# td-kwj-zp2023/webgpu-msm-bls12-377

Measured on AMD Instinct MI355X. Metric: ms per 2^20 BLS12-377 G1 MSM, lower is better.
Workload: dtype u32 (29-bit limbs, 64-bit accumulate)

## Files before the change

### webgpu-msm-bls12-377_amd/csrc/capi.hip

```cpp
#include <hip/hip_runtime.h>
#include <stdlib.h>
#include <string.h>

#include <algorithm>
#include <new>

#include "context.hpp"
#include "host_tail.hpp"
#include "sequencer.hpp"
#include "batch_mul_host.hpp"
#include "import_host.hpp"
#include "validate_host.hpp"

using namespace msm377;

#define HIP_TRY(ctx, call)                                                  \
  do {                                                                      \
    if (!eng::hip_ok((ctx), (int)(call), #call)) return MSM377_EHIP;        \
  } while (0)


extern "C" {

const char* msm377_version(void) { return "msm377 0.1 gfx950"; }

const char* msm377_strerror(int code) {
  switch (code) {
    case MSM377_OK: return "ok";
    case MSM377_EINVAL: return "invalid argument";
    case MSM377_EHIP: return "HIP runtime error";
    case MSM377_ESCALAR: return "scalar out of range for the signed window recode";
    case MSM377_ENOMEM: return "out of memory";
    case MSM377_ESTATE: return "call sequence error";
    case MSM377_EGLVRANGE: return "scalar outside the GLV range";
    case MSM377_EEXCEPTIONAL: return "exceptional case of the twisted Edwards law while combining partial records";
    case MSM377_EPOINT: return "an input point failed a requested check (canonical / on the curve / in the subgroup)";
    default: return "unknown error";
  }
}

int msm377_ctx_create(int device, uint64_t max_points, msm377_ctx** out) {
  if (!out || max_points == 0 || max_points > (1ull << 30)) return MSM377_EINVAL;
  *out = nullptr;
  int count = 0;
  if (hipGetDeviceCount(&count) != hipSuccess || device < 0 || device >= count) return MSM377_EHIP;
  msm377_ctx* ctx = new (std::nothrow) msm377_ctx();
  if (!ctx) return MSM377_ENOMEM;
  ctx->device = device;
  ctx->cap = max_points;
  if (const char* e = getenv("MSM377_GLV")) ctx->glv_mode = atoi(e);
  if (const char* e = getenv("MSM377_G1_FORM")) ctx->g1_form = atoi(e) != 0;
  if (const char* e = getenv("MSM377_CONV_WAVE_PRIO")) ctx->conv_wave_prio = atoi(e) != 0;
  if (const char* e = getenv("MSM377_AFF_PREWAKE_US")) ctx->aff_prewake_us = atoll(e);
  if (const char* e = getenv("MSM377_UPLOAD_CHUNKS")) ctx->upload_chunks = (uint32_t)std::min(std::max(atoi(e), 2), 7);
  if (const char* e = getenv("MSM377_UPLOAD_SPLIT")) ctx->upload_split_pct = (uint32_t)std::min(std::max(atoi(e), 5), 90);
  if (const char* e = getenv("MSM377_UPLOAD_CHUNK_MIN")) ctx->upload_chunk_min = strtoull(e, nullptr, 10);
  if (const char* e = getenv("MSM377_TAIL_THREADS")) ctx->tail_threads = std::min(std::max(atoi(e), 1), TailPool::WORKERS + 1);
  if (const char* e = getenv("MSM377_TAIL_WAIT_MS")) ctx->tail_pool.wait_limit_ns = (int64_t)std::max(atoi(e), 1) * 1000000ll;
  if (const char* e = getenv("MSM377_TAIL_SPIN_US")) ctx->tail_spin_us = atoll(e);
  if (const char* e = getenv("MSM377_TAIL_TRACE")) ctx->tail_trace = atoi(e) != 0;
  if (const char* e = getenv("MSM377_TAIL_NUMA")) ctx->tail_pool.numa_local = atoi(e) != 0;
  if (const char* e = getenv("MSM377_TE_AFFINE_MSM")) ctx->te_affine_msm = atoi(e) != 0;
  if (const char* e = getenv("MSM377_NARROW_MAX")) ctx->narrow_max_points = strtoull(e, nullptr, 10);
  if (const char* e = getenv("MSM377_PRECOMP_BITS")) ctx->precomp_bits = atoi(e) == (int)WIDE_BITS ? (int)WIDE_BITS : MSM377_WINDOW_BITS;
  if (const char* e = getenv("MSM377_AFFINE_MIN")) ctx->affine_min_points = strtoull(e, nullptr, 10);
  if (const char* e = getenv("MSM377_SEG_PLAIN")) ctx->seg_plain = std::min(std::max(atoi(e), (int)SEG_MIN), (int)SEG_MAX);
  if (const char* e = getenv("MSM377_SEG_GLV")) ctx->seg_glv = std::min(std::max(atoi(e), (int)SEG_MIN), (int)SEG_MAX);
  if (const char* e = getenv("MSM377_ZERO_COPY_OUT")) ctx->zc_out = atoi(e);
  if (const char* e = getenv("MSM377_NARROW_SEG")) ctx->narrow_seg = (uint32_t)std::min(std::max(atoi(e), (int)NARROW_SEG), (int)SEG_BINS - 1);
  if (const char* e = getenv("MSM377_NARROW_QUAD_ITEMS")) ctx->narrow_quad_items = strtoull(e, nullptr, 10);
  if (const char* e = getenv("MSM377_COOP_THREADS")) ctx->coop_threads = (uint32_t)atoi(e);
  if (const char* e = getenv("MSM377_NARROW_TAIL_FROM")) ctx->narrow_tail_from = (uint32_t)std::min(std::max(atoi(e), 1), (int)TREE_LEVELS);
  if (const char* e = getenv("MSM377_TAIL_LDS")) ctx->tail_lds = atoi(e) != 0;
  if (const char* e = getenv("MSM377_REDUCE_COLUMNS")) ctx->reduce_columns = atoi(e) != 0;
  if (const char* e = getenv("MSM377_EVEN_WINDOWS")) ctx->even_windows = atoi(e) != 0;
  if (const char* e = getenv("MSM377_SORT_ELEM")) ctx->sort_elem = atoi(e) == 4 ? 4u : 8u;
  if (const char* e = getenv("MSM377_TWIN_BATCH")) ctx->twin_batches = atoi(e) != 0;
  if (const char* e = getenv("MSM377_BASE_CHECKS")) ctx->base_checks = check_flags_normal((uint32_t)strtoul(e, nullptr, 0));
  if (const char* e = getenv("MSM377_TAIL_FROM")) ctx->tail_from = (uint32_t)std::min(std::max(atoi(e), 1), (int)TREE_LEVELS);
  const uint64_t cap = max_points;
  int prio_least = 0, prio_greatest = 0;
  bool ok = hipSetDevice(device) == hipSuccess;
  if (ok && hipDeviceGetStreamPriorityRange(&prio_least, &prio_greatest) != hipSuccess) prio_least = prio_greatest = 0;
  ok = ok && hipStreamCreateWithPriority(&ctx->stream, hipStreamNonBlocking, prio_greatest) == hipSuccess &&
            hipStreamCreateWithPriority(&ctx->stream2, hipStreamNonBlocking, prio_least) == hipSuccess &&
            hipEventCreateWithFlags(&ctx->bases_ready, hipEventDisableTiming) == hipSuccess;
  auto dalloc = [&](void** p, size_t bytes) { ok = ok && hipMalloc(p, bytes) == hipSuccess; };
  dalloc((void**)&ctx->d_raw_points, cap * 96);
  dalloc((void**)&ctx->d_raw_scalars, cap * 32);
  dalloc((void**)&ctx->d_bases, 2 * cap * G1_REC_WORDS * 4);
  const uint64_t wcap = std::max<uint64_t>((uint64_t)MSM377_NUM_WINDOWS * cap, (uint64_t)NARROW_EVEN_WINDOWS * std::min<uint64_t>(cap, SMALL_SORT_MAX));
  dalloc((void**)&ctx->d_digits, wcap * 2);
  dalloc((void**)&ctx->d_range_counts, (size_t)NRANGE * MAX_SORT_BLOCKS * 4);
  dalloc((void**)&ctx->d_region_base, (size_t)MSM377_NUM_WINDOWS * (NRANGE + 1) * 4);
  dalloc((void**)&ctx->d_sort_temp, cap * MSM377_NUM_WINDOWS * sizeof(SortElem));
  dalloc((void**)&ctx->d_row_ptr, (size_t)MSM377_NUM_WINDOWS * RP * 4);
  dalloc((void**)&ctx->d_val_idx, wcap * 4);
  dalloc((void**)&ctx->d_buckets, (size_t)MSM377_NUM_WINDOWS * BKT_WORDS * NB * 4);
  dalloc((void**)&ctx->d_partials, (size_t)2 * SLOT_WORDS * 4);
  const uint64_t extra_items = std::max<uint64_t>((uint64_t)MSM377_NUM_WINDOWS * cap / SEG_MIN, (uint64_t)NARROW_EVEN_WINDOWS * std::min<uint64_t>(cap, SMALL_SORT_MAX) / NARROW_SEG) + 2;
  dalloc((void**)&ctx->d_work, ((size_t)MSM377_NUM_WINDOWS * NB + extra_items) * sizeof(WorkItem));
  dalloc((void**)&ctx->d_work_meta, (size_t)META_BLOCK_WORDS * 4);
  dalloc((void**)&ctx->d_row_ovf_base, (size_t)MSM377_NUM_WINDOWS * NB * 4);
  dalloc((void**)&ctx->d_split_rows, (size_t)MSM377_NUM_WINDOWS * NB * 4);
  dalloc((void**)&ctx->d_ovf, (size_t)extra_items * BKT_WORDS * 4);
  const size_t aff_blocks = (size_t)affine_blocks(cap) + 1;
  dalloc((void**)&ctx->d_aff_count, 64);
  ok = ok && hipMemset(ctx->d_aff_count, 0, 64) == hipSuccess;
  dalloc((void**)&ctx->d_aff_stash, (size_t)affine_blocks(cap) * AFF_BLOCK_POINTS * AFF_STASH_WORDS * 4);
  dalloc((void**)&ctx->d_aff_trees, aff_blocks * 2 * AFF_THREADS * 13 * 4);
  const unsigned host_flags = hipHostMallocMapped | hipHostMallocCoherent;
  ok = ok && hipHostMalloc((void**)&ctx->h_aff_prod, aff_blocks * 48, host_flags) == hipSuccess &&
       hipHostMalloc((void**)&ctx->h_aff_inv, aff_blocks * 48, host_flags) == hipSuccess &&
       hipHostMalloc((void**)&ctx->h_aff_flag, 64, host_flags) == hipSuccess &&
       hipHostGetDevicePointer((void**)&ctx->dm_aff_prod, ctx->h_aff_prod, 0) == hipSuccess &&
       hipHostGetDevicePointer((void**)&ctx->dm_aff_inv, ctx->h_aff_inv, 0) == hipSuccess &&
       hipHostGetDevicePointer((void**)&ctx->dm_aff_flag, ctx->h_aff_flag, 0) == hipSuccess &&
       hipEventCreateWithFlags(&ctx->aff_up_done, hipEventDisableTiming) == hipSuccess;
  if (ok) ctx->aff_scratch.resize(aff_blocks);
  dalloc((void**)&ctx->d_err, 4 * sizeof(int));
  ok = ok && hipHostMalloc((void**)&ctx->h_partials, (size_t)2 * SLOT_WORDS * 4, host_flags) == hipSuccess &&
       hipHostGetDevicePointer((void**)&ctx->dm_partials, ctx->h_partials, 0) == hipSuccess &&
       hipHostMalloc((void**)&ctx->h_out_flag, 64, host_flags) == hipSuccess &&
       hipHostGetDevicePointer((void**)&ctx->dm_out_flag, ctx->h_out_flag, 0) == hipSuccess;
  if (ok) memset(ctx->h_out_flag, 0, 64);
  dalloc((void**)&ctx->d_out_count, 64);
  ok = ok && hipMemset(ctx->d_out_count, 0, 64) == hipSuccess;
  ok = ok && hipHostMalloc((void**)&ctx->h_err, 2 * sizeof(int)) == hipSuccess;
  for (int k = 0; ok && k < 2; k++) ok = ok && hipEventCreateWithFlags(&ctx->done_ev[k], hipEventDisableTiming) == hipSuccess;
  for (int s = 0; ok && s < MSM377_NUM_STAGES; s++)
    for (int k = 0; k < 2; k++) ok = ok && hipEventCreate(&ctx->ev[s][k]) == hipSuccess;
  if (!ok) {
    msm377_ctx_destroy(ctx);
    return MSM377_ENOMEM;
  }
  *out = ctx;
  return MSM377_OK;
}

void msm377_ctx_destroy(msm377_ctx* ctx) {
  if (!ctx) return;
  ctx->tail_pool.shutdown();
  (void)hipSetDevice(ctx->device);
  if (ctx->stream) (void)hipStreamSynchronize(ctx->stream);
  if (ctx->stream2) (void)hipStreamSynchronize(ctx->stream2);
  if (ctx->twin) {
    eng::twin_return(ctx);
    msm377_ctx_destroy(ctx->twin);
    ctx->twin = nullptr;
  }
  void* bufs[] = {ctx->d_raw_points, ctx->d_raw_scalars, ctx->d_bases, ctx->d_digits, ctx->d_range_counts, ctx->d_region_base, ctx->d_sort_temp,
                  ctx->d_row_ptr, ctx->d_val_idx, ctx->d_buckets, ctx->d_buckets_snap, ctx->d_partials, ctx->d_work, ctx->d_work_meta, ctx->d_row_ovf_base, ctx->d_split_rows, ctx->d_ovf, ctx->d_err, ctx->d_aff_stash, ctx->d_aff_trees, ctx->d_aff_count, ctx->d_out_count, ctx->resident.table, ctx->d_native, ctx->d_inf_mask,
                  ctx->bm.table, ctx->bm.stash, ctx->bm.trees, ctx->bm.block_prod, ctx->bm.block_inv, ctx->bm.row_bases, ctx->bm.base_wire};
  for (void* p : bufs)
    if (p) (void)hipFree(p);
  ctx->wide.release();
  if (ctx->h_partials) (void)hipHostFree(ctx->h_partials);
  if (ctx->h_err) (void)hipHostFree(ctx->h_err);
  if (ctx->h_out_flag) (void)hipHostFree(ctx->h_out_flag);
  if (ctx->h_stage) (void)hipHostFree(ctx->h_stage);
  if (ctx->h_aff_prod) (void)hipHostFree(ctx->h_aff_prod);
  if (ctx->h_aff_inv) (void)hipHostFree(ctx->h_aff_inv);
  if (ctx->h_aff_flag) (void)hipHostFree(ctx->h_aff_flag);
  if (ctx->aff_up_done) (void)hipEventDestroy(ctx->aff_up_done);
  if (ctx->import_done) (void)hipEventDestroy(ctx->import_done);
  for (int t = 0; t < 8; t++)
    if (ctx->copy_stream[t]) (void)hipStreamDestroy(ctx->copy_stream[t]);
  for (int k = 0; k < 2; k++)
    if (ctx->done_ev[k]) (void)hipEventDestroy(ctx->done_ev[k]);
  for (int s = 0; s < MSM377_NUM_STAGES; s++)
    for (int k = 0; k < 2; k++)
      if (ctx->ev[s][k]) (void)hipEventDestroy(ctx->ev[s][k]);
  if (ctx->bases_ready) (void)hipEventDestroy(ctx->bases_ready);
  if (ctx->stream2) (void)hipStreamDestroy(ctx->stream2);
  if (ctx->stream) (void)hipStreamDestroy(ctx->stream);
  delete ctx;
}

const char* msm377_last_error(const msm377_ctx* ctx) { return ctx ? ctx->err.c_str() : "null context"; }














int msm377_g1_window_partials_device(msm377_ctx* ctx, const void* d_points, const void* d_scalars, uint64_t n, uint32_t win_begin,
                                     uint32_t win_count, uint8_t* partials_out) {
  if (!partials_out) return MSM377_EINVAL;
  return eng::window_partials(ctx, d_points, d_scalars, n, win_begin, win_count, partials_out, nullptr);
}

int msm377_g1_window_partials_resident(msm377_ctx* ctx, const void* d_points, const void* d_scalars, uint64_t n, uint32_t win_begin,
                                       uint32_t win_count, void* d_partials_out) {
  if (!d_partials_out) return MSM377_EINVAL;
  return eng::window_partials(ctx, d_points, d_scalars, n, win_begin, win_count, nullptr, d_partials_out);
}


int msm377_g1_combine_window_partials(const uint8_t* partials, uint32_t num_windows, uint8_t out_xy[96]) {
  if (!partials || !out_xy || ((uintptr_t)partials & 3) || num_windows == 0 || num_windows > MSM377_NUM_WINDOWS) return MSM377_EINVAL;
  return g1_combine_tagged(reinterpret_cast<const uint32_t*>(partials), (int)num_windows, out_xy) ? MSM377_EEXCEPTIONAL : MSM377_OK;
}

int msm377_g1_combine_partials_ctx(msm377_ctx* ctx, const uint8_t* partials, uint8_t out_xy[96]) {
  if (!ctx || !partials || !out_xy || ((uintptr_t)partials & 3)) return MSM377_EINVAL;
  const uint32_t* rec = reinterpret_cast<const uint32_t*>(partials);
  bool all_te = true, all_w = true;
  for (int w = 0; w < MSM377_NUM_WINDOWS; w++) {
    const bool te = window_record_is_te(rec + (size_t)w * MSM377_G1_PARTIAL_POINTS * MSM377_G1_POINT_WORDS);
    all_te = all_te && te;
    all_w = all_w && !te;
  }
  int rc = MSM377_OK;
  if (all_te)
    {
    const int tr = eng::te_tail(ctx, rec, out_xy);
    rc = tr == eng::TAIL_EXCEPTIONAL ? MSM377_EEXCEPTIONAL : tr;
  }
  else if (all_w)
    rc = eng::xyzz_tail(ctx, rec, out_xy);
  else
    rc = g1_combine_tagged(rec, MSM377_NUM_WINDOWS, out_xy) ? MSM377_EEXCEPTIONAL : MSM377_OK;
  if (rc == MSM377_EEXCEPTIONAL) ctx->err = "the partial records add up to an exceptional case of the twisted Edwards law (points outside the prime-order subgroup): recompute them in form 0";
  return rc;
}

int msm377_g1_fold_window_partials(uint8_t* partials, uint32_t win_count) {
  if (!partials || ((uintptr_t)partials & 3) || win_count > MSM377_NUM_WINDOWS) return MSM377_EINVAL;
  g1_fold_tagged(reinterpret_cast<uint32_t*>(partials), (int)win_count);
  return MSM377_OK;
}

int msm377_g1_combine_partials(const uint8_t* partials, uint8_t out_xy[96]) {
  if (!partials || !out_xy || ((uintptr_t)partials & 3)) return MSM377_EINVAL;
  return g1_combine_tagged(reinterpret_cast<const uint32_t*>(partials), MSM377_NUM_WINDOWS, out_xy) ? MSM377_EEXCEPTIONAL : MSM377_OK;
}

int msm377_g1_add_points(const uint8_t* points_xy, uint32_t count, uint8_t out_xy[96]) {
  if (!out_xy || (count && !points_xy)) return MSM377_EINVAL;
  return g1h_add_wire_points(points_xy, count, out_xy) ? MSM377_OK : MSM377_EINVAL;
}

int msm377_g1_combine_partials_split(const uint8_t* partials, uint32_t pieces, uint8_t out_xy[96]) {
  if (!partials || !out_xy || ((uintptr_t)partials & 3) || pieces < 1 || pieces > 64) return MSM377_EINVAL;
  const uint32_t* p = reinterpret_cast<const uint32_t*>(partials);
  for (int w = 0; w < MSM377_NUM_WINDOWS; w++)
    if (!window_record_is_te(p + (size_t)w * 16 * 48)) return MSM377_EINVAL;
  return teh_combine_split(p, MSM377_NUM_WINDOWS, out_xy, (int)pieces) ? MSM377_EEXCEPTIONAL : MSM377_OK;
}


int msm377_ctx_set_stage_capture(msm377_ctx* ctx, int enabled) {
  if (!ctx || enabled < 0 || enabled > 2) return MSM377_EINVAL;
  if (enabled && !ctx->d_buckets_snap) {
    HIP_TRY(ctx, hipSetDevice(ctx->device));
    if (hipMalloc((void**)&ctx->d_buckets_snap, (size_t)MSM377_NUM_WINDOWS * BKT_WORDS * NB * 4) != hipSuccess) return MSM377_ENOMEM;
  }
  ctx->capture = enabled;
  ctx->stage.valid = false;
  return MSM377_OK;
}

int msm377_g1_read_stage(msm377_ctx* ctx, uint32_t slot, uint16_t* digits, uint32_t* row_ptr, uint32_t* val_idx, uint32_t* buckets) {
  if (!ctx) return MSM377_EINVAL;
  if (ctx->capture != 1 || ctx->last_n == 0 || slot >= ctx->last_wc || ctx->last_form < 0 || ctx->last_glv) {
    ctx->err = "no captured stage data for that window slot (capture mode 2 is read with msm377_g1_read_stage_ex)";
    return MSM377_ESTATE;
  }
  HIP_TRY(ctx, hipSetDevice(ctx->device));
  const uint64_t n = ctx->last_n;
  if (digits) HIP_TRY(ctx, hipMemcpy(digits, ctx->d_digits + (size_t)slot * n, n * 2, hipMemcpyDeviceToHost));
  if (row_ptr) HIP_TRY(ctx, hipMemcpy(row_ptr, ctx->d_row_ptr + (size_t)slot * RP, RP * 4, hipMemcpyDeviceToHost));
  if (val_idx) HIP_TRY(ctx, hipMemcpy(val_idx, ctx->d_val_idx + (size_t)slot * n, n * 4, hipMemcpyDeviceToHost));
  if (buckets) {
    uint32_t* tmp = (uint32_t*)malloc((size_t)BKT_WORDS * NB * 4);
    if (!tmp) return MSM377_ENOMEM;
    hipError_t e = hipMemcpy(tmp, ctx->d_buckets_snap + (size_t)slot * BKT_WORDS * NB, (size_t)BKT_WORDS * NB * 4, hipMemcpyDeviceToHost);
    if (e == hipSuccess)
      for (uint32_t t = 0; t < NB; t++)
        for (uint32_t c = 0; c < 4; c++)
          for (uint32_t j = 0; j < 13; j++) buckets[(size_t)t * PT_WORDS + c * 13 + j] = tmp[(size_t)t * BKT_WORDS + c * 16 + j];
    free(tmp);
    HIP_TRY(ctx, e);
  }
  return MSM377_OK;
}

int msm377_g1_read_stage_ex(msm377_ctx* ctx, uint32_t slot, msm377_stage_info* info, void* digits, uint32_t* row_ptr, uint32_t* val_idx, uint32_t* buckets) {
  if (!ctx) return MSM377_EINVAL;
  const StageLayout& sl = ctx->stage;
  if (!ctx->capture || !sl.valid || !ctx->d_buckets_snap) {
    ctx->err = "no captured stage data: stage capture is off, or the last call is not one the capture mode describes";
    return MSM377_ESTATE;
  }
  if (slot >= sl.info.slots) {
    ctx->err = "no captured stage data for that window slot";
    return MSM377_ESTATE;
  }
  HIP_TRY(ctx, hipSetDevice(ctx->device));
  msm377_stage_info out = sl.info;
  if (sl.d_key_max) {
    uint32_t words[MSM377_NUM_WINDOWS] = {};
    HIP_TRY(ctx, hipMemcpy(words, sl.d_key_max, sizeof words, hipMemcpyDeviceToHost));
    for (uint32_t s = 0; s < out.slots && s < MSM377_NUM_WINDOWS; s++) out.key_max[s] = words[s];
  }
  if (info) *info = out;
  const uint64_t cols = out.columns;
  const size_t records = out.bucket_records;
  if (digits) HIP_TRY(ctx, hipMemcpy(digits, (const uint8_t*)sl.d_digits + (size_t)slot * cols * out.digit_bytes, cols * out.digit_bytes, hipMemcpyDeviceToHost));
  if (row_ptr) HIP_TRY(ctx, hipMemcpy(row_ptr, ctx->d_row_ptr + (size_t)slot * out.row_ptr_len, (size_t)out.row_ptr_len * 4, hipMemcpyDeviceToHost));
  if (val_idx) HIP_TRY(ctx, hipMemcpy(val_idx, ctx->d_val_idx + (size_t)slot * cols, cols * 4, hipMemcpyDeviceToHost));
  if (buckets) {
    uint32_t* tmp = (uint32_t*)malloc(records * BKT_WORDS * 4);
    if (!tmp) return MSM377_ENOMEM;
    hipError_t e = hipMemcpy(tmp, ctx->d_buckets_snap + (size_t)slot * records * BKT_WORDS, records * BKT_WORDS * 4, hipMemcpyDeviceToHost);
    if (e == hipSuccess)
      for (size_t t = 0; t < records; t++)
        for (uint32_t c = 0; c < 4; c++)
          for (uint32_t j = 0; j < 13; j++) buckets[t * PT_WORDS + c * 13 + j] = tmp[t * BKT_WORDS + c * 16 + j];
    free(tmp);
    HIP_TRY(ctx, e);
  }
  return MSM377_OK;
}

int msm377_ctx_get_stage_form(const msm377_ctx* ctx) { return (ctx && ctx->capture && ctx->last_n) ? ctx->last_form : -1; }

int msm377_g1_xyzz_to_affine(const uint32_t xyzz[52], uint8_t out_xy[96]) {
  if (!xyzz || !out_xy) return MSM377_EINVAL;
  g1h_to_wire(g1h_from_device_words(xyzz), out_xy);
  return MSM377_OK;
}

int msm377_ctx_set_glv(msm377_ctx* ctx, int mode) {
  if (!ctx || mode < 0 || mode > 2) return MSM377_EINVAL;
  ctx->glv_mode = mode == 1 ? 1 : 0;
  return MSM377_OK;
}

int msm377_ctx_set_g1_form(msm377_ctx* ctx, int form) {
  if (!ctx || form < 0 || form > 1) return MSM377_EINVAL;
  ctx->g1_form = form;
  return MSM377_OK;
}

int msm377_ctx_get_products_per_addition(const msm377_ctx* ctx) { return ctx ? ctx->last_products : 0; }

int msm377_ctx_get_fallback_info(const msm377_ctx* ctx, uint64_t* count, uint32_t* last_mask) {
  if (!ctx) return MSM377_EINVAL;
  if (count) *count = ctx->fallback_count;
  if (last_mask) *last_mask = ctx->fallback_mask;
  return MSM377_OK;
}

int msm377_ctx_set_precompute_window(msm377_ctx* ctx, int window_bits) {
  if (!ctx || (window_bits != MSM377_WINDOW_BITS && window_bits != MSM377_WIDE_WINDOW_BITS)) return MSM377_EINVAL;
  ctx->precomp_bits = window_bits;
  return MSM377_OK;
}

int msm377_ctx_set_base_checks(msm377_ctx* ctx, uint32_t flags) {
  if (!ctx || (flags && !check_flags_normal(flags))) return MSM377_EINVAL;
  ctx->base_checks = check_flags_normal(flags);
  return MSM377_OK;
}

int msm377_ctx_set_input_format(msm377_ctx* ctx, uint32_t point_form, uint32_t scalar_form) {
  if (!ctx || point_form > MSM377_POINTS_MONT_FLAG || scalar_form > MSM377_SCALARS_MONT) return MSM377_EINVAL;
  ctx->point_form = point_form;
  ctx->scalar_form = scalar_form;
  return MSM377_OK;
}

int msm377_ctx_get_input_format(const msm377_ctx* ctx, uint32_t* point_form, uint32_t* scalar_form) {
  if (!ctx) return MSM377_EINVAL;
  if (point_form) *point_form = ctx->point_form;
  if (scalar_form) *scalar_form = ctx->scalar_form;
  return MSM377_OK;
}

int msm377_g1_import_points_host(const uint8_t* in, uint64_t n, uint32_t point_form, uint8_t* out_wire, uint32_t* out_inf_mask) {
  if (point_form > MSM377_POINTS_MONT_FLAG || (n && (!in || !out_wire))) return MSM377_EINVAL;
  import_points_host(in, n, point_form, out_wire, out_inf_mask);
  return MSM377_OK;
}

int msm377_import_scalars_host(const uint8_t* in, uint64_t n, uint32_t scalar_form, uint8_t* out_wire) {
  if (scalar_form > MSM377_SCALARS_MONT || (n && (!in || !out_wire))) return MSM377_EINVAL;
  import_scalars_host(in, n, scalar_form, out_wire);
  return MSM377_OK;
}

int msm377_g1_result_to_native(const uint8_t xy[96], uint8_t out[104]) {
  if (!xy || !out) return MSM377_EINVAL;
  return result_to_native_host(xy, out) ? MSM377_OK : MSM377_EINVAL;
}

int msm377_g1_batch_mul_host(const uint8_t base_xy[96], const uint8_t* scalars, uint64_t n, uint32_t out_form, uint8_t* out_points, uint8_t* out_inf) {
  return batch_mul_host(base_xy, scalars, n, MSM377_SCALARS_WIRE, out_form, out_points, out_inf);
}

int msm377_ctx_set_mul_window(msm377_ctx* ctx, int window_bits) {
  if (!ctx || (window_bits != 0 && !batch_mul_width_supported(window_bits))) return MSM377_EINVAL;
  ctx->bm.window = window_bits;
  return MSM377_OK;
}

int msm377_ctx_get_last_mul_window(const msm377_ctx* ctx) { return ctx ? ctx->bm.last_window : 0; }

uint64_t msm377_ctx_get_mul_table_builds(const msm377_ctx* ctx) { return ctx ? ctx->bm.builds : 0; }

int msm377_ctx_get_last_check(const msm377_ctx* ctx, msm377_check_report* out) {
  if (!ctx || !out) return MSM377_EINVAL;
  *out = ctx->last_check;
  return MSM377_OK;
}

static int check_host_args(const uint8_t* points, uint64_t n, uint32_t flags, msm377_check_report* out) {
  return (!out || !check_flags_normal(flags) || (n && !points)) ? MSM377_EINVAL : MSM377_OK;
}
int msm377_g1_check_points_host(const uint8_t* points, uint64_t n, uint32_t flags, msm377_check_report* out) {
  if (check_host_args(points, n, flags, out)) return MSM377_EINVAL;
  check_points_host<G1HostCheck>(points, n, check_flags_normal(flags), out);
  return MSM377_OK;
}
int msm377_ed_check_points_host(const uint8_t* points, uint64_t n, uint32_t flags, msm377_check_report* out) {
  if (check_host_args(points, n, flags, out)) return MSM377_EINVAL;
  check_points_host<EdHostCheck>(points, n, check_flags_normal(flags), out);
  return MSM377_OK;
}

uint32_t msm377_short_windows(uint32_t scalar_bits, uint32_t bucket_log) {
  if (scalar_bits < 1 || scalar_bits > 253 || bucket_log < 1 || bucket_log > 15) return 0;
  return short_windows(scalar_bits, bucket_log);
}

int msm377_scalars_width_host(const uint8_t* scalars, uint64_t n, uint32_t scalar_bytes, uint32_t* bits_out) {
  if (!bits_out || (n && !scalars) || (scalar_bytes != 4 && scalar_bytes != 8 && scalar_bytes != 16 && scalar_bytes != 32)) return MSM377_EINVAL;
  uint32_t best = 0;
  for (uint64_t i = 0; i < n; i++) {
    const uint8_t* k = scalars + i * scalar_bytes;
    for (uint32_t j = scalar_bytes; j-- > 0;) {
      if (!k[j]) continue;
      const uint32_t len = 8 * j + 32 - (uint32_t)__builtin_clz((uint32_t)k[j]);
      best = std::max(best, len);
      break;
// ... 67 lines not shown
```

### webgpu-msm-bls12-377_amd/csrc/common.hpp

```cpp
#pragma once
#include <stdint.h>

#include "../../include/msm377.h"

#ifndef MSM_HD
#if defined(__HIPCC__)
#include <hip/hip_runtime.h>
#define MSM_HD __host__ __device__ __forceinline__
#else
#define MSM_HD inline __attribute__((always_inline))
#endif
#endif

namespace msm377 {

constexpr uint32_t NB = 32768;
constexpr uint32_t NBIN = NB + 1;
constexpr uint32_t RP = NBIN + 1;
constexpr uint32_t PT_WORDS = 52;
constexpr uint32_t BKT_WORDS = 64;
constexpr uint32_t MAX_SORT_BLOCKS = 256;
constexpr uint32_t TREE_LEVELS = 15;
constexpr uint32_t SEG_MIN = 16;
constexpr uint32_t SEG_MAX = 128;
constexpr uint32_t SEG_BINS = SEG_MAX + 1;
constexpr int ERR_SCALAR = 1, ERR_GLV_RANGE = 2, ERR_NARROW_RANGE = 128;
constexpr int ERR_SHORT_WIDTH = 256;
constexpr int ERR_TE_EXCEPTIONAL = MSM377_FB_ACCUMULATE, ERR_TE_MERGE = MSM377_FB_MERGE, ERR_TE_TREE = MSM377_FB_TREE, ERR_TE_CONVERT = MSM377_FB_CONVERT;
constexpr int ERR_TE_ANY = ERR_TE_EXCEPTIONAL | ERR_TE_MERGE | ERR_TE_TREE | ERR_TE_CONVERT;
constexpr uint32_t NARROW_LOG = 11;
constexpr uint32_t NARROW_SEG = 8;
constexpr uint32_t NARROW_EVEN_WINDOWS = 22, NARROW_EVEN_SIGNED = 11, NARROW_EVEN_BITS = NARROW_LOG + 1;
static_assert(NARROW_EVEN_SIGNED * NARROW_EVEN_BITS + (NARROW_EVEN_WINDOWS - NARROW_EVEN_SIGNED) * NARROW_LOG == 253, "the windows cover a 253-bit scalar");
constexpr uint32_t MAX_WINDOW_SLOTS = NARROW_EVEN_WINDOWS > MSM377_NUM_WINDOWS ? NARROW_EVEN_WINDOWS : MSM377_NUM_WINDOWS;

constexpr uint32_t short_windows(uint32_t bits, uint32_t L) { return bits / (L + 1) + 1; }
static_assert(short_windows(253, 15) == MSM377_NUM_WINDOWS && short_windows(253, NARROW_LOG) == NARROW_EVEN_WINDOWS, "at full width: the window counts of the main and the narrow path");

constexpr uint32_t NRANGE = 256;
constexpr uint32_t KRANGE = NB / NRANGE;
constexpr uint32_t KEY_TRACKED = 0x80000000u;
constexpr uint32_t KEY_UNSIGNED = 0x40000000u;
constexpr uint32_t SMALL_SORT_MAX = 1u << 16;
constexpr uint32_t SMALL_BINS_MAX = (1u << 12) + 1;
struct SortElem {
  uint32_t idx_sign;
  uint32_t key;
};
struct SortElem4 {
  uint32_t v;
};
constexpr uint32_t SORT_IDX_BITS = 23, SORT_SUB_BITS = 8;
constexpr uint64_t SORT_PACKED_MAX_COLUMNS = 1ull << SORT_IDX_BITS;
static_assert(SORT_IDX_BITS + SORT_SUB_BITS + 1 == 32, "index, sub and sign fill the 32-bit element");
static_assert(KRANGE < (1u << SORT_SUB_BITS), "sub = 0..KRANGE fits its field");
MSM_HD SortElem4 sort_pack(uint32_t idx, uint32_t sign, uint32_t sub) { return SortElem4{(sign << 31) | (sub << SORT_IDX_BITS) | idx}; }
MSM_HD uint32_t sort_sub(SortElem4 e) { return (e.v >> SORT_IDX_BITS) & ((1u << SORT_SUB_BITS) - 1u); }
MSM_HD uint32_t sort_idx_sign(SortElem4 e) { return e.v & ~(((1u << SORT_SUB_BITS) - 1u) << SORT_IDX_BITS); }
MSM_HD uint32_t range_first_key(uint32_t rg, uint32_t shift) { return rg * (KRANGE >> shift); }
inline uint32_t sort_elem_bytes(uint64_t columns, bool wide) { return (!wide && columns <= SORT_PACKED_MAX_COLUMNS) ? 4u : 8u; }

struct WorkItem {
  uint32_t row;
  uint32_t seg;
};
constexpr uint32_t META_BLOCK_WORDS = 2 * SEG_BINS + 4 + MSM377_NUM_WINDOWS;
constexpr size_t SLOT_WORDS = (size_t)MAX_WINDOW_SLOTS * MSM377_G1_PARTIAL_POINTS * MSM377_G1_POINT_WORDS;

constexpr uint32_t AFF_THREADS = 256, AFF_K = 8, AFF_BLOCK_POINTS = AFF_THREADS * AFF_K;
constexpr uint32_t AFF_STASH_WORDS = 52;
inline uint32_t affine_blocks(uint64_t n) { return (uint32_t)((n + AFF_BLOCK_POINTS - 1) / AFF_BLOCK_POINTS); }

constexpr uint32_t ACC_FLAG_WORD = 4;
constexpr uint32_t EVEN_FROM = 13;
constexpr uint32_t even_offset(uint32_t w) { return 16 * w - (w > EVEN_FROM ? w - EVEN_FROM : 0u); }
static_assert(even_offset(13) == 208 && even_offset(14) == 223 && even_offset(15) == 238 && even_offset(16) == 253, "13 x 16 + 3 x 15 = 253 bits");
constexpr uint32_t WIDE_BITS = MSM377_WIDE_WINDOW_BITS;
constexpr uint32_t WIDE_LOG = 19;
constexpr uint32_t WIDE_WINDOWS = 13;
constexpr uint32_t WIDE_FULL = 6;
constexpr uint32_t wide_width(uint32_t w) { return w < WIDE_FULL ? WIDE_BITS : WIDE_BITS - 1; }
constexpr uint32_t wide_offset(uint32_t w) { return w <= WIDE_FULL ? WIDE_BITS * w : WIDE_BITS * WIDE_FULL + (WIDE_BITS - 1) * (w - WIDE_FULL); }
static_assert(wide_offset(WIDE_WINDOWS - 1) == 234 && wide_offset(WIDE_WINDOWS - 1) + wide_width(WIDE_WINDOWS - 1) == 253, "the windows cover a 253-bit scalar");
constexpr uint32_t WIDE_NRANGE = 4096;
constexpr uint32_t WIDE_POINTS = WIDE_LOG + 1;
static_assert((1u << WIDE_LOG) == WIDE_NRANGE * KRANGE, "ranges of KRANGE keys cover the wide bucket set");
static_assert((1u << WIDE_LOG) <= MSM377_NUM_WINDOWS * NB, "the wide bucket set fits the main path's bucket, row and work-list buffers");
static_assert(WIDE_POINTS * 1 <= MAX_WINDOW_SLOTS * MSM377_G1_PARTIAL_POINTS, "the wide window record fits a partial-record slot");

constexpr uint32_t G1_REC_WORDS = 32;
constexpr uint32_t GLV_WINDOWS = MSM377_GLV_WINDOWS;

}
```

### webgpu-msm-bls12-377_amd/csrc/context.hpp

```cpp
#pragma once
#include <hip/hip_runtime.h>

#include <functional>
#include <string>
#include <vector>

#include "common.hpp"
#include "fp64_host.hpp"
#include "tail_pool.hpp"

using msm377::SortElem;
using msm377::WorkItem;
using msm377::TailPool;
using msm377::Fp64;
using msm377::MAX_WINDOW_SLOTS;
using msm377::NARROW_SEG;

struct ResidentBases {
  uint64_t n = 0;
  int form = 0;
  uint32_t* bases = nullptr;
  uint32_t* table = nullptr;
  uint64_t cap = 0;
  uint32_t windows = 0;
  uint32_t flagged = 0;
  const uint32_t* inf_mask = nullptr;
  bool valid() const { return n != 0; }
  void clear() { n = 0; flagged = 0; }
  void set(uint32_t* records, uint64_t count, int table_form, uint32_t flagged_points = 0, const uint32_t* mask = nullptr) {
    bases = records; n = count; form = table_form; flagged = flagged_points; inf_mask = mask;
  }
};

struct BatchMulState {
  int window = 0;
  int last_window = 0;
  uint64_t builds = 0;
  bool valid = false;
  uint8_t base[96] = {};
  int width = 0;
  uint32_t* table = nullptr;
  uint64_t table_cap = 0;
  uint32_t* stash = nullptr;
  uint32_t* trees = nullptr;
  uint32_t* block_prod = nullptr;
  uint32_t* block_inv = nullptr;
  uint32_t* row_bases = nullptr;
  uint32_t* base_wire = nullptr;
};

struct WideBuffers {
  uint32_t* digits = nullptr;
  SortElem* temp = nullptr;
  uint32_t* counts = nullptr;
  uint64_t cap = 0;
  bool ensure(uint64_t n);
  void release() {
    for (void* p : {(void*)digits, (void*)temp, (void*)counts}) (void)hipFree(p);
    *this = WideBuffers();
  }
};

struct StageLayout {
  bool valid = false;
  msm377_stage_info info = {};
  const void* d_digits = nullptr;
  const uint32_t* d_key_max = nullptr;
};

struct msm377_ctx {
  int device = 0;
  hipStream_t stream = nullptr;
  hipStream_t stream2 = nullptr;
  hipEvent_t bases_ready = nullptr;
  uint64_t cap = 0;
  std::string err;
  uint32_t* d_raw_points = nullptr;
  uint32_t* d_raw_scalars = nullptr;
  uint32_t* d_bases = nullptr;
  uint16_t* d_digits = nullptr;
  uint32_t* d_range_counts = nullptr;
  uint32_t* d_region_base = nullptr;
  SortElem* d_sort_temp = nullptr;
  uint32_t* d_row_ptr = nullptr;
  uint32_t* d_val_idx = nullptr;
  uint32_t* d_buckets = nullptr;
  uint32_t* d_buckets_snap = nullptr;
  uint32_t* d_partials = nullptr;
  WorkItem* d_work = nullptr;
  uint32_t* d_work_meta = nullptr;
  uint32_t* d_row_ovf_base = nullptr;
  uint32_t* d_split_rows = nullptr;
  uint32_t* d_ovf = nullptr;
  uint32_t point_form = MSM377_POINTS_WIRE, scalar_form = MSM377_SCALARS_WIRE;
  uint8_t* d_native = nullptr;
  uint32_t* d_inf_mask = nullptr;
  hipEvent_t import_done = nullptr;
  ResidentBases resident;
  BatchMulState bm;
  WideBuffers wide;
  int precomp_bits = MSM377_WINDOW_BITS;
  uint32_t* d_aff_stash = nullptr;
  uint32_t* d_aff_trees = nullptr;
  uint32_t* h_aff_prod = nullptr;
  uint32_t* h_aff_inv = nullptr;
  uint32_t* h_aff_flag = nullptr;
  uint32_t *dm_aff_prod = nullptr, *dm_aff_inv = nullptr, *dm_aff_flag = nullptr;
  uint32_t* d_aff_count = nullptr;
  hipEvent_t aff_up_done = nullptr;
  std::vector<Fp64::El> aff_scratch;
  bool te_affine_msm = true;
  uint64_t affine_min_points = 1ull << 20;
  int* d_err = nullptr;
  uint32_t* h_partials = nullptr;
  int* h_err = nullptr;
  hipEvent_t done_ev[2] = {};
  uint8_t* h_stage = nullptr;
  hipStream_t copy_stream[8] = {};
  uint64_t last_n = 0;
  uint32_t last_wc = 0;
  uint32_t last_geom_windows = 0, last_geom_log = 0;
  uint32_t last_sort_elem = 0;
  int last_form = -1;
  int capture = 0;
  StageLayout stage;
  int zc_out = 1;
  bool zc_active = false;
  uint32_t out_seq = 0;
  uint32_t* h_out_flag = nullptr;
  uint32_t* dm_out_flag = nullptr;
  uint32_t* dm_partials = nullptr;
  uint32_t* d_out_count = nullptr;
  int timing = 0;
  uint32_t coop_threads = 131072;
  uint32_t narrow_tail_from = 4;
  uint32_t narrow_seg = 0;
  uint64_t narrow_quad_items = 100000;
  uint32_t tail_from = 7;
  bool reduce_columns = true;
  int glv_mode = 0;
  int g1_form = 1;
  bool last_glv = false;
  uint32_t seg_plain = 0, seg_glv = 0;
  hipEvent_t ev[MSM377_NUM_STAGES][2] = {};
  uint64_t upload_chunk_min = 1ull << 18;
  uint32_t upload_chunks = 4;
  uint32_t upload_split_pct = 30;
  std::function<int()> before_accumulate;
  TailPool tail_pool;
  int tail_threads = 6;
  int64_t aff_prewake_us = 600;
  uint32_t conv_wave_prio = 1;
  int64_t tail_spin_us = 1000;
  bool tail_trace = false;
  double stage_ms[MSM377_NUM_STAGES] = {};
  int last_products = 0;
  uint64_t narrow_max_points = 1ull << 16;
  bool tail_lds = true;
  bool even_windows = true;
  uint32_t sort_elem = 8;
  bool ed_equal_windows_once = false;
  uint32_t acc_seq = 0;
  msm377_ctx* twin = nullptr;
  bool twin_batches = true;
  bool twin_failed = false;
  uint32_t base_checks = 0;
  msm377_check_report last_check = {0, 0, 0, 0, UINT64_MAX, 0, 0};
  uint64_t fallback_count = 0;
  uint64_t geometry_reruns = 0;
  uint32_t fallback_mask = 0;
};
```

### webgpu-msm-bls12-377_amd/csrc/kernels/accumulate.hpp

```cpp
#pragma once
#include "../curves.hpp"
#include "reduce.hpp"

namespace msm377 {
namespace {



__device__ __forceinline__ const uint32_t* row_bounds(const uint32_t* __restrict__ row_ptr, uint32_t L, uint32_t ws, uint32_t t) {
  return row_ptr + (size_t)ws * ((1u << L) + 2) + t + 1;
}
__device__ __forceinline__ uint32_t row_len(const uint32_t* __restrict__ row_ptr, uint32_t L, uint32_t row) {
  const int at = (int)(row + 2 * (row >> L) + 1);
  return row_ptr[at + 1] - row_ptr[at];
}

struct RowSplit {
  uint32_t nseg, seglen, lastlen;
};
__device__ __forceinline__ RowSplit row_split(uint32_t len, uint32_t SEG) {
  RowSplit r;
  if (len <= SEG) {
    r.nseg = 1;
    r.seglen = r.lastlen = len;
    return r;
  }
  const uint32_t parts = (len + SEG - 1) / SEG;
  r.seglen = (len + parts - 1) / parts;
  r.nseg = (len + r.seglen - 1) / r.seglen;
  r.lastlen = len - (r.nseg - 1) * r.seglen;
  return r;
}

__global__ void __launch_bounds__(1024) k_work_hist(const uint32_t* __restrict__ row_ptr, uint32_t L, uint32_t rows, uint32_t SEG, uint32_t* __restrict__ work_hist,
                                                   uint32_t* __restrict__ row_ovf_base, uint32_t* __restrict__ counters ,
                                                   uint32_t* __restrict__ split_rows) {
  __shared__ uint32_t lh[SEG_BINS];
  __shared__ uint32_t blk[4];
  const uint32_t tid = threadIdx.x, row = blockIdx.x * 1024 + tid;
  if (tid < SEG_BINS) lh[tid] = 0;
  if (tid < 2) blk[tid] = 0;
  __syncthreads();
  RowSplit sp = {1, 0, 0};
  uint32_t my_split = 0, my_ovf = 0;
  if (row < rows) {
    sp = row_split(row_len(row_ptr, L, row), SEG);
    atomicAdd(&lh[sp.lastlen], 1u);
    if (sp.nseg > 1) {
      atomicAdd(&lh[sp.seglen], sp.nseg - 1);
      my_split = atomicAdd(&blk[0], 1u);
      my_ovf = atomicAdd(&blk[1], sp.nseg - 1);
    }
  }
  __syncthreads();
  if (tid < SEG_BINS && lh[tid]) atomicAdd(&work_hist[tid], lh[tid]);
  if (tid == 0 && blk[0]) {
    blk[2] = atomicAdd(&counters[0], blk[0]);
    blk[3] = atomicAdd(&counters[1], blk[1]);
  }
  __syncthreads();
  if (sp.nseg > 1) {
    row_ovf_base[row] = blk[3] + my_ovf;
    split_rows[blk[2] + my_split] = row;
  }
}

__global__ void __launch_bounds__(1024) k_work_scatter(const uint32_t* __restrict__ row_ptr, uint32_t L, uint32_t rows, uint32_t SEG,
                                                      const uint32_t* __restrict__ work_hist, uint32_t* __restrict__ cursor, uint32_t* __restrict__ total,
                                                      WorkItem* __restrict__ work) {
  __shared__ uint32_t lh[SEG_BINS];
  __shared__ uint32_t lbase[SEG_BINS];
  __shared__ uint32_t gh[SEG_BINS];
  const uint32_t tid = threadIdx.x, row = blockIdx.x * 1024 + tid;
  if (tid < SEG_BINS) {
    lh[tid] = 0;
    gh[tid] = work_hist[tid];
  }
  __syncthreads();
  uint32_t first = 0;
  if (tid < SEG_BINS) {
    for (uint32_t b = tid + 1; b < SEG_BINS; b++) first += gh[b];
    if (tid == 0 && blockIdx.x == 0) *total = first + gh[0];
  }
  RowSplit sp = {0, 0, 0};
  uint32_t rank_full = 0, rank_last = 0;
  if (row < rows) {
    sp = row_split(row_len(row_ptr, L, row), SEG);
    if (sp.nseg > 1) rank_full = atomicAdd(&lh[sp.seglen], sp.nseg - 1);
    rank_last = atomicAdd(&lh[sp.lastlen], 1u);
  }
  __syncthreads();
  if (tid < SEG_BINS && lh[tid]) lbase[tid] = first + atomicAdd(&cursor[tid], lh[tid]);
  __syncthreads();
  if (row < rows) {
    for (uint32_t s = 0; s + 1 < sp.nseg; s++) work[lbase[sp.seglen] + rank_full + s] = WorkItem{row, s};
    work[lbase[sp.lastlen] + rank_last] = WorkItem{row, sp.nseg - 1};
  }
}

template <class T>
__device__ __forceinline__ void pin_registers(T& o) {
  static_assert(sizeof(T) % 4 == 0, "whole words");
  uint32_t w[sizeof(T) / 4];
  __builtin_memcpy(w, &o, sizeof(T));
#pragma unroll
  for (int j = 0; j < (int)(sizeof(T) / 4); j++) asm volatile("" : "+v"(w[j]));
  __builtin_memcpy(&o, w, sizeof(T));
}

template <class CV, int OCC, class BP = CV, int PF = 0>
__global__ void __launch_bounds__(256, OCC) k_accumulate(const uint32_t* __restrict__ row_ptr, const uint32_t* __restrict__ val_idx,
                                                       const uint32_t* __restrict__ bases, uint32_t* __restrict__ buckets, uint64_t n,
                                                       const WorkItem* __restrict__ work, const uint32_t* __restrict__ work_total,
                                                       const uint32_t* __restrict__ row_ovf_base, uint32_t* __restrict__ ovf, uint32_t SEG,
                                                       int* __restrict__ err, const int* __restrict__ conv_err, uint32_t into, uint64_t table_stride, uint32_t L) {
  const uint32_t v = blockIdx.x * 256 + threadIdx.x;
  if (v == 0 && *conv_err) atomicOr(err, *conv_err);
  if (v >= *work_total) return;
  const WorkItem it = work[v];
  const uint32_t ws = it.row >> L, t = it.row & ((1u << L) - 1);
  const uint32_t* rb = row_bounds(row_ptr, L, ws, t);
  const uint32_t* vi = val_idx + (size_t)ws * n;
  bases += (size_t)ws * table_stride * BP::REC_WORDS;
  const uint32_t row_beg = rb[0], row_end = rb[1];
  const uint32_t seglen = row_split(row_end - row_beg, SEG).seglen;
  uint32_t k = row_beg + it.seg * seglen;
  const uint32_t end = (row_end - k > seglen) ? k + seglen : row_end;
  typename CV::Pt acc = (into && it.seg == 0) ? load_bucket<CV>(buckets, L, ws, t) : CV::identity();
  const bool start_fresh = !(into && it.seg == 0);
  bool bad = false;
  if (k < end) {
    static_assert(PF == 0, "one record in flight");
    uint32_t e_cur = vi[k];
    uint32_t e_nxt = (k + 1 < end) ? vi[k + 1] : 0u;
    typename BP::Base rec = BP::load_base(bases, e_cur & 0x7fffffffu);
    bool more = true;
    auto advance = [&]() {
      k++;
      more = k < end;
      if (more) {
        rec = BP::load_base(bases, e_nxt & 0x7fffffffu);
        e_cur = e_nxt;
        e_nxt = (k + 1 < end) ? vi[k + 1] : 0u;
      }
    };
    auto stage = [&](auto first_tag) {
      constexpr bool FIRST = decltype(first_tag)::value;
      const bool neg = (e_cur >> 31) != 0;
      if constexpr (FIRST) {
        const typename BP::Base cur = rec;
        advance();
        acc = BP::first(cur, neg);
      } else {
        typename BP::Ops ops = BP::signed_ops(rec, neg);
        pin_registers(ops);
        advance();
        acc = BP::madd(acc, ops);
      }
      bad |= CV::is_bad(acc);
    };
    if (start_fresh) stage(std::true_type{});
    while (more) stage(std::false_type{});
  }
  if (bad) atomicOr(err, ERR_TE_EXCEPTIONAL);
  if (it.seg == 0) {
    store_bucket<CV>(buckets, L, ws, t, acc);
  } else {
    store_record<CV>(ovf + (size_t)(row_ovf_base[it.row] + it.seg - 1) * CV::BKT_WORDS, acc);
  }
}

template <class F, class K>
__device__ __forceinline__ typename TeLazy<F, K>::Ext te_madd_quad(const typename TeLazy<F, K>::Ext& a, const typename F::El& mine, uint32_t q) {
  using El = typename F::El;
  const El m1 = F::mul_lz(sel4(q, F::add_kp_sub(a.y, K::KP2, a.x), F::add_lz(a.y, a.x), a.t, a.z), mine);
  const El pa = quad_bcast<0>(m1), pb = quad_bcast<1>(m1), c = quad_bcast<2>(m1), d = quad_bcast<3>(m1);
  const El e = F::norm(F::add_kp_sub(pb, K::KP2, pa)), f = F::norm(F::add_kp_sub(d, K::KP2, c));
  const El g = F::norm(F::add_lz(d, c)), h = F::add_lz(pb, pa);
  const El m3 = F::mul_lz(sel4(q, e, h, h, f), sel4(q, f, g, e, g));
  typename TeLazy<F, K>::Ext o;
  o.x = quad_bcast<0>(m3);
  o.y = quad_bcast<1>(m3);
  o.t = quad_bcast<2>(m3);
  o.z = quad_bcast<3>(m3);
  return o;
}

template <class CV>
__global__ void __launch_bounds__(256, 2) k_accumulate_quad(const uint32_t* __restrict__ row_ptr, const uint32_t* __restrict__ val_idx,
                                                          const uint32_t* __restrict__ bases, uint32_t* __restrict__ buckets, uint64_t n,
                                                          const WorkItem* __restrict__ work, const uint32_t* __restrict__ work_total,
                                                          const uint32_t* __restrict__ row_ovf_base, uint32_t* __restrict__ ovf, uint32_t SEG,
                                                          int* __restrict__ err, const int* __restrict__ conv_err, uint32_t into, uint32_t L) {
  using El = typename CV::F::El;
  using K = typename CV::Pt_K;
  const uint32_t gid = blockIdx.x * 256 + threadIdx.x;
  const uint32_t v = gid >> 2, q = threadIdx.x & 3;
  if (gid == 0 && *conv_err) atomicOr(err, *conv_err);
  if (v >= *work_total) return;
  const WorkItem it = work[v];
  const uint32_t ws = it.row >> L, t = it.row & ((1u << L) - 1);
  const uint32_t* rb = row_bounds(row_ptr, L, ws, t);
  const uint32_t* vi = val_idx + (size_t)ws * n;
  const uint32_t row_beg = rb[0], row_end = rb[1];
  const uint32_t seglen = row_split(row_end - row_beg, SEG).seglen;
  uint32_t k = row_beg + it.seg * seglen;
  const uint32_t end = (row_end - k > seglen) ? k + seglen : row_end;
  const bool continues = into && it.seg == 0;
  typename CV::Pt acc = continues ? load_bucket<CV>(buckets, L, ws, t) : CV::identity();
  bool bad = false;
  auto load_mine = [&](uint32_t e) {
    const bool neg = (e >> 31) != 0;
    const uint32_t comp = q < 2 ? (q ^ (neg ? 1u : 0u)) : q;
    const uint32_t* src = bases + (size_t)(e & 0x7fffffffu) * CV::REC_WORDS + comp * CV::NL;
    El r;
#pragma unroll
    for (int j = 0; j < (int)CV::NL; j++) r.l[j] = src[j];
    return r;
  };
  if (k < end && !continues) {
    const uint32_t e = vi[k];
    acc = CV::first(CV::load_base(bases, e & 0x7fffffffu), (e >> 31) != 0);
    bad |= CV::is_bad(acc);
    k++;
  }
  if (k < end) {
    uint32_t e_cur = vi[k];
    uint32_t e_nxt = (k + 1 < end) ? vi[k + 1] : 0u;
    El cur = load_mine(e_cur);
    for (;;) {
      k++;
      const bool more = k < end;
      El nxt = cur;
      uint32_t e_nn = 0u;
      if (more) {
        nxt = load_mine(e_nxt);
        if (k + 1 < end) e_nn = vi[k + 1];
      }
      const El mine = (q == 2 && (e_cur >> 31)) ? CV::F::kp_sub(K::KP2, cur) : cur;
      acc = te_madd_quad<typename CV::F, K>(acc, mine, q);
      bad |= CV::is_bad(acc);
      if (!more) break;
      cur = nxt;
      e_cur = e_nxt;
      e_nxt = e_nn;
    }
  }
  if (bad) atomicOr(err, ERR_TE_EXCEPTIONAL);
  uint32_t* dst = it.seg == 0 ? bucket_ptr<CV>(buckets, L, ws, t) : ovf + (size_t)(row_ovf_base[it.row] + it.seg - 1) * CV::BKT_WORDS;
  store_coord<CV>(dst + q * CV::COORD_WORDS, coord4(q, acc).l);
}

constexpr uint32_t OVF_FOLDED = 0x80000000u;
constexpr uint32_t LONG_ROW_PARTIALS = 32, FOLD_THREADS = 512, FOLD_BLOCKS = 64;
static_assert((1u << 15) <= FOLD_THREADS * FOLD_BLOCKS, "one pass of the grid sees every row of a window (L <= 15)");
template <class CV>
__global__ void __launch_bounds__(FOLD_THREADS) k_fold_long_rows(const uint32_t* __restrict__ row_ptr, uint32_t* __restrict__ row_ovf_base, uint32_t* __restrict__ ovf,
                                                                 uint32_t SEG, int* __restrict__ err, uint32_t L, uint32_t ws) {
  __shared__ uint32_t list[FOLD_THREADS];
  __shared__ uint32_t nlist;
  if (threadIdx.x == 0) nlist = 0;
  __syncthreads();
  {
    const uint32_t t = blockIdx.x + gridDim.x * threadIdx.x;
    if (t < (1u << L) && row_split(row_len(row_ptr, L, (ws << L) + t), SEG).nseg > LONG_ROW_PARTIALS) list[atomicAdd(&nlist, 1u)] = (ws << L) + t;
  }
  __syncthreads();
  const uint32_t q = threadIdx.x & 3, quad = threadIdx.x >> 2;
  bool bad = false;
  for (uint32_t i = 0; i < nlist; i++) {
    const uint32_t row = list[i];
    uint32_t* rec = ovf + (size_t)row_ovf_base[row] * CV::BKT_WORDS;
    for (uint32_t cur = row_split(row_len(row_ptr, L, row), SEG).nseg - 1; cur > 1;) {
      const uint32_t half = (cur + 1) / 2;
      for (uint32_t j = quad; j + half < cur; j += FOLD_THREADS / 4) {
        uint32_t* a = rec + (size_t)j * CV::BKT_WORDS;
        const typename CV::Pt sum = add_quad(load_record_quad<CV>(a, q), load_record_quad<CV>(rec + (size_t)(j + half) * CV::BKT_WORDS, q), q);
        bad |= CV::is_bad(sum);
        store_coord<CV>(a + q * CV::COORD_WORDS, coord4(q, sum).l);
      }
      cur = half;
      __syncthreads();
    }
  }
  __syncthreads();
  for (uint32_t i = threadIdx.x; i < nlist; i += FOLD_THREADS) row_ovf_base[list[i]] |= OVF_FOLDED;
  if (bad) atomicOr(err, ERR_TE_MERGE);
}

template <class CV>
__global__ void __launch_bounds__(256, 2) k_merge_split_rows_quad(const uint32_t* __restrict__ row_ptr, uint32_t* __restrict__ buckets,
                                                                  const uint32_t* __restrict__ counters, const uint32_t* __restrict__ split_rows,
                                                                  const uint32_t* __restrict__ row_ovf_base, const uint32_t* __restrict__ ovf, uint32_t SEG,
                                                                  int* __restrict__ err, uint32_t L, uint32_t* __restrict__ host_flag, uint32_t seq) {
  if (host_flag && blockIdx.x == 0 && threadIdx.x == 0) __hip_atomic_store(host_flag, seq, __ATOMIC_RELAXED, __HIP_MEMORY_SCOPE_SYSTEM);
  const uint32_t count = counters[0];
  const uint32_t q = threadIdx.x & 3;
  for (uint32_t i = (blockIdx.x * 256 + threadIdx.x) >> 2; i < count; i += gridDim.x * 64) {
    const uint32_t row = split_rows[i];
    const uint32_t len = row_len(row_ptr, L, row);
    const uint32_t ovf_at = row_ovf_base[row];
    const uint32_t nseg = (ovf_at & OVF_FOLDED) ? 2u : row_split(len, SEG).nseg;
    const uint32_t ws = row >> L, t = row & ((1u << L) - 1);
    typename CV::Pt acc = load_bucket_quad<CV>(buckets, L, ws, t, q);
    const uint32_t* src = ovf + (size_t)(ovf_at & ~OVF_FOLDED) * CV::BKT_WORDS;
    typename CV::Pt nxt = load_record_quad<CV>(src, q);
    bool bad = false;
    for (uint32_t s = 1; s < nseg; s++) {
      const typename CV::Pt cur = nxt;
      if (s + 1 < nseg) nxt = load_record_quad<CV>(src + (size_t)s * CV::BKT_WORDS, q);
      acc = add_quad(acc, cur, q);
      bad |= CV::is_bad(acc);
    }
    if (bad) atomicOr(err, ERR_TE_MERGE);
    const typename CV::F::El c = coord4(q, acc);
    store_coord<CV>(bucket_ptr<CV>(buckets, L, ws, t) + q * CV::COORD_WORDS, c.l);
  }
}

}
}
```

### webgpu-msm-bls12-377_amd/csrc/kernels/convert.hpp

```cpp
#pragma once
#include "../curves.hpp"

namespace msm377 {
namespace {


__global__ void __launch_bounds__(256) k_clear_words(uint32_t* __restrict__ a, uint32_t na, uint32_t* __restrict__ b, uint32_t nb) {
  for (uint32_t i = threadIdx.x; i < na; i += 256) a[i] = 0;
  for (uint32_t i = threadIdx.x; i < nb; i += 256) b[i] = 0;
}

template <class CV>
__global__ void __launch_bounds__(256) k_convert_bases(const uint32_t* __restrict__ raw, uint32_t* __restrict__ bases, uint64_t n, int* __restrict__ err) {
  uint64_t i = (uint64_t)blockIdx.x * 256 + threadIdx.x;
  if (i >= n) return;
  uint32_t w[CV::RAW_WORDS];
  load_words16(raw + i * CV::RAW_WORDS, w, CV::RAW_WORDS / 4);
  uint32_t o[CV::REC_WORDS];
  if (CV::convert(w, o)) atomicOr(err, ERR_TE_CONVERT);
  uint4* dst = reinterpret_cast<uint4*>(bases + i * CV::REC_WORDS);
#pragma unroll
  for (int k = 0; k < (int)CV::REC_WORDS / 4; k++) dst[k] = make_uint4(o[4 * k], o[4 * k + 1], o[4 * k + 2], o[4 * k + 3]);
}


__device__ __forceinline__ void put13(uint32_t* w, const Fp::El& e) {
#pragma unroll
  for (int j = 0; j < 13; j++) w[j] = e.l[j];
}
__device__ __forceinline__ Fp::El get13(const uint32_t* w) {
  Fp::El e;
#pragma unroll
  for (int j = 0; j < 13; j++) e.l[j] = w[j];
  return e;
}
struct AffWireSource {
  const uint32_t* raw;
  __device__ __forceinline__ bool load(uint64_t i, Fp::El& n1, Fp::El& n2, Fp::El& z) const {
    using K = G1Consts;
    uint32_t w[24];
    load_words16(raw + i * 24, w, 6);
    const Fp::El xr = Fp::from_words<12>(w), yr = Fp::from_words<12>(w + 12);
    const Fp::El u = Fp::add_lz(Fp::mul_lz(xr, Fp::from_const(K::TE_SR)), Fp::from_const(K::TE_S));
    const Fp::El v = Fp::mul_lz(yr, Fp::from_const(K::TE_SR));
    const Fp::El cu = Fp::csub(Fp::norm(Fp::add_lz(Fp::mul_lz(xr, Fp::from_const(K::TE_CSR)), Fp::from_const(K::TE_CS))), K::MOD);
    const Fp::El up = Fp::add_lz(u, Fp::one());
    z = Fp::mul_lz(up, v);
    n1 = Fp::mul_lz(up, cu);
    n2 = Fp::norm(Fp::add_kp_sub_sub2(z, K::KP4W3, Fp::zero(), v));
    return Te377::is_zero_mod_p(z);
  }
};
struct AffDoublingSource {
  const uint32_t* prev;
  uint32_t bits;
  __device__ __forceinline__ bool load(uint64_t i, Fp::El& n1, Fp::El& n2, Fp::El& z) const {
    Te377::Ext p = Te377::from_base_affine(TeAffBase::load_base(prev, (uint32_t)i), false);
    bool bad = false;
#pragma unroll 1
    for (uint32_t k = 0; k < bits; k++) {
      p = Te377::add(p, p);
      bad |= Te377::is_bad(p);
    }
    n1 = Fp::canon(p.x);
    n2 = Fp::canon(p.y);
    z = Fp::canon(p.z);
    return bad;
  }
};
template <class SRC>
__global__ void __launch_bounds__(AFF_THREADS, 4) k_affine_up(SRC src, uint64_t n, uint32_t* __restrict__ stash,
                                                              uint32_t* __restrict__ trees, uint32_t* __restrict__ block_prod, uint32_t* __restrict__ host_flag, uint32_t* __restrict__ dev_count,
                                                              int* __restrict__ err, uint32_t prio) {
  if (prio) __builtin_amdgcn_s_setprio(3);
  using K = G1Consts;
  __shared__ uint32_t tree[2 * AFF_THREADS][13];
  const uint32_t tid = threadIdx.x, blk = blockIdx.x;
  const uint64_t base = (uint64_t)blk * AFF_BLOCK_POINTS + tid;
  bool bad = false;
  Fp::El c = Fp::one();
#pragma unroll 1
  for (uint32_t j = 0; j < AFF_K; j++) {
    const uint64_t i = base + (uint64_t)j * AFF_THREADS;
    if (i >= n) break;
    Fp::El n1, n2, z;
    if (src.load(i, n1, n2, z)) {
      bad = true;
      z = Fp::one();
    }
    uint32_t o[AFF_STASH_WORDS];
    put13(o, n1);
    put13(o + 13, n2);
    put13(o + 26, z);
    put13(o + 39, c);
    uint4* dst = reinterpret_cast<uint4*>(stash) + ((size_t)blk * AFF_K + j) * (AFF_STASH_WORDS / 4) * AFF_THREADS + tid;
#pragma unroll
    for (int k = 0; k < (int)AFF_STASH_WORDS / 4; k++) dst[(size_t)k * AFF_THREADS] = make_uint4(o[4 * k], o[4 * k + 1], o[4 * k + 2], o[4 * k + 3]);
    c = Fp::mul_lz(c, z);
  }
  if (bad) atomicOr(err, ERR_TE_CONVERT);
  put13(tree[AFF_THREADS + tid], c);
  for (uint32_t size = AFF_THREADS / 2; size >= 1; size >>= 1) {
    __syncthreads();
    if (tid < size) put13(tree[size + tid], Fp::mul_lz(get13(tree[2 * (size + tid)]), get13(tree[2 * (size + tid) + 1])));
  }
  __syncthreads();
  uint32_t* out = trees + (size_t)blk * (2 * AFF_THREADS * 13);
  const uint32_t* flat = &tree[0][0];
  for (uint32_t k = tid; k < 2 * AFF_THREADS * 13; k += AFF_THREADS) out[k] = flat[k];
  if (tid == 0) {
    const Fp::El root = Fp::mul(get13(tree[1]), Fp::from_const(K::TO64));
    uint32_t w[12];
    Fp::to_words<12>(root, w);
#pragma unroll
    for (int j = 0; j < 12; j++) block_prod[(size_t)blk * 12 + j] = w[j];
    __threadfence_system();
    if (atomicAdd(dev_count, 1u) == gridDim.x - 1) {
      *dev_count = 0;
      __threadfence_system();
      *reinterpret_cast<volatile uint32_t*>(host_flag) = gridDim.x;
    }
  }
}

__global__ void __launch_bounds__(AFF_THREADS, 2) k_affine_down(uint64_t n, const uint32_t* __restrict__ stash, const uint32_t* __restrict__ trees,
                                                                const uint32_t* __restrict__ block_inv, uint32_t* __restrict__ bases, uint32_t prio) {
  if (prio) __builtin_amdgcn_s_setprio(3);
  __shared__ uint32_t tree[2 * AFF_THREADS][13];
  const uint32_t tid = threadIdx.x, blk = blockIdx.x;
  const uint32_t* in = trees + (size_t)blk * (2 * AFF_THREADS * 13);
  uint32_t* flat = &tree[0][0];
  for (uint32_t k = tid; k < 2 * AFF_THREADS * 13; k += AFF_THREADS) flat[k] = in[k];
  __syncthreads();
  if (tid == 0) {
    uint32_t w[12];
#pragma unroll
    for (int j = 0; j < 12; j++) w[j] = block_inv[(size_t)blk * 12 + j];
    put13(tree[1], Fp::from_words<12>(w));
  }
  for (uint32_t size = 1; size < AFF_THREADS; size <<= 1) {
    __syncthreads();
    if (tid < size) {
      const uint32_t k = size + tid;
      const Fp::El inv_k = get13(tree[k]), a = get13(tree[2 * k]), b = get13(tree[2 * k + 1]);
      put13(tree[2 * k], Fp::mul_lz(inv_k, b));
      put13(tree[2 * k + 1], Fp::mul_lz(inv_k, a));
    }
  }
  __syncthreads();
  Fp::El inv = get13(tree[AFF_THREADS + tid]);
  const uint64_t base = (uint64_t)blk * AFF_BLOCK_POINTS + tid;
#pragma unroll 1
  for (int j = (int)AFF_K - 1; j >= 0; j--) {
    const uint64_t i = base + (uint64_t)j * AFF_THREADS;
    if (i >= n) continue;
    uint32_t w[AFF_STASH_WORDS];
    {
      const uint4* src = reinterpret_cast<const uint4*>(stash) + ((size_t)blk * AFF_K + j) * (AFF_STASH_WORDS / 4) * AFF_THREADS + tid;
#pragma unroll
      for (int k = 0; k < (int)AFF_STASH_WORDS / 4; k++) {
        const uint4 v = src[(size_t)k * AFF_THREADS];
        w[4 * k + 0] = v.x;
        w[4 * k + 1] = v.y;
        w[4 * k + 2] = v.z;
        w[4 * k + 3] = v.w;
      }
    }
    const Fp::El zi = Fp::mul_lz(inv, get13(w + 39));
    inv = Fp::mul_lz(inv, get13(w + 26));
    const Fp::El x = Fp::mul(get13(w), zi), y = Fp::mul(get13(w + 13), zi);
    const Fp::El ymx = Fp::sub(y, x), ypx = Fp::add(y, x), kt = Fp::mul_lz(Fp::mul_lz(x, y), Fp::from_const(G1Consts::TE_2D));
    uint32_t o[TeAffBase::REC_WORDS];
    put13(o, ymx);
    put13(o + 13, ypx);
    put13(o + 26, kt);
    o[39] = 0;
    uint4* dst = reinterpret_cast<uint4*>(bases + i * TeAffBase::REC_WORDS);
#pragma unroll
    for (int k = 0; k < (int)TeAffBase::REC_WORDS / 4; k++) dst[k] = make_uint4(o[4 * k], o[4 * k + 1], o[4 * k + 2], o[4 * k + 3]);
  }
}


__global__ void __launch_bounds__(256) k_convert_bases_glv(const uint32_t* __restrict__ raw, uint32_t* __restrict__ bases, uint64_t n) {
  uint64_t i = (uint64_t)blockIdx.x * 256 + threadIdx.x;
  if (i >= n) return;
  uint32_t w[24];
  load_words16(raw + i * 24, w, 6);
  const Fp::El x = Fp::to_mont(Fp::from_words<12>(w));
  const Fp::El y = Fp::to_mont(Fp::from_words<12>(w + 12));
  const Fp::El bx = Fp::mul(x, Fp::from_const(G1Consts::BETA));
  constexpr uint32_t REC_WORDS = G1Dev::REC_WORDS;
  uint32_t o[REC_WORDS];
#pragma unroll
  for (int j = 0; j < 13; j++) {
    o[j] = x.l[j];
    o[13 + j] = y.l[j];
  }
#pragma unroll
  for (int j = 26; j < 32; j++) o[j] = 0;
  uint4* dst = reinterpret_cast<uint4*>(bases + i * REC_WORDS);
#pragma unroll
  for (int k = 0; k < 8; k++) dst[k] = make_uint4(o[4 * k], o[4 * k + 1], o[4 * k + 2], o[4 * k + 3]);
#pragma unroll
  for (int j = 0; j < 13; j++) o[j] = bx.l[j];
  dst = reinterpret_cast<uint4*>(bases + (n + i) * REC_WORDS);
#pragma unroll
  for (int k = 0; k < 8; k++) dst[k] = make_uint4(o[4 * k], o[4 * k + 1], o[4 * k + 2], o[4 * k + 3]);
}


}
}
```

### webgpu-msm-bls12-377_amd/csrc/kernels/decompose.hpp

```cpp
#pragma once
#include "../curves.hpp"

namespace msm377 {
namespace {

__device__ __forceinline__ void digit_key(uint32_t biased, uint32_t& key, uint32_t& sign) {
  int d = (int)biased - 32768;
  sign = d < 0 ? 1u : 0u;
  key = (uint32_t)(d < 0 ? -d : d);
}
__device__ __forceinline__ void digit_key(uint32_t stored, bool uns, uint32_t& key, uint32_t& sign) {
  digit_key(stored, key, sign);
  if (uns) key = stored, sign = 0u;
}
__device__ __forceinline__ uint32_t win_shift(uint32_t key_max_word) {
  if (!(key_max_word & KEY_TRACKED)) return 0;
  const uint32_t max_key = key_max_word & ~(KEY_TRACKED | KEY_UNSIGNED);
  uint32_t s = 0;
  while (s < 5 && max_key < (NB >> (s + 1))) s++;
  return s;
}
__device__ __forceinline__ uint32_t key_range(uint32_t key, uint32_t s) {
  return s == 0 ? (key >= NB ? NRANGE - 1 : key / KRANGE) : key >> (7 - s);
}

__global__ void __launch_bounds__(256) k_decompose(const uint32_t* __restrict__ scalars, uint16_t* __restrict__ digits, uint64_t n,
                                                   uint32_t wb, uint32_t wc, int* __restrict__ err, uint32_t* __restrict__ top_key_max, uint32_t even) {
  __shared__ uint32_t wmax;
  if (threadIdx.x == 0) wmax = 0;
  __syncthreads();
  uint64_t i = (uint64_t)blockIdx.x * 256 + threadIdx.x;
  if (i < n) {
    uint32_t w[8];
    load_words16(scalars + i * 8, w, 2);
    uint32_t carry = 0;
    if (even) {
      uint32_t carry16 = 0;
#pragma unroll
      for (uint32_t win = 0; win < 16; win++) {
        const uint32_t limb = (w[win >> 1] >> (16 * (win & 1))) & 0xffffu;
        carry16 = limb + carry16 >= 32768u ? 1u : 0u;
        uint32_t biased;
        if (win < EVEN_FROM) {
          const uint32_t v = limb + carry;
          carry = v >= 32768u ? 1u : 0u;
          biased = (v + 32768u) & 0xffffu;
        } else {
          const uint32_t raw = win == 13 ? (w[6] >> 16) & 0x7fffu : win == 14 ? (w[6] >> 31) | ((w[7] & 0x3fffu) << 1) : (w[7] >> 14) & 0x7fffu;
          const uint32_t v = raw + carry;
          carry = v >> 15;
          biased = (v & 0x7fffu) + 32768u;
        }
        if (win >= wb && win < wb + wc) digits[(size_t)(win - wb) * n + i] = (uint16_t)biased;
      }
      if (carry | (w[7] >> 29)) atomicOr(err, ERR_NARROW_RANGE);
      if (carry16) atomicOr(err, ERR_SCALAR);
    } else {
#pragma unroll
      for (uint32_t win = 0; win < 16; win++) {
        uint32_t limb = (w[win >> 1] >> (16 * (win & 1))) & 0xffffu;
        uint32_t v = limb + carry;
        carry = v >= 32768u ? 1u : 0u;
        if (win >= wb && win < wb + wc) {
          const uint32_t biased = (v + 32768u) & 0xffffu;
          digits[(size_t)(win - wb) * n + i] = (uint16_t)biased;
          if (win == 15 && top_key_max) {
            uint32_t key, sign;
            digit_key(biased, key, sign);
            if ((key | KEY_TRACKED) > wmax) atomicMax(&wmax, key | KEY_TRACKED);
          }
        }
      }
      if (carry) atomicOr(err, 1);
    }
  }
  __syncthreads();
  if (threadIdx.x == 0 && top_key_max && wmax > *top_key_max) atomicMax(top_key_max, wmax);
}


__global__ void __launch_bounds__(256) k_decompose_geom(const uint32_t* __restrict__ scalars, uint16_t* __restrict__ digits, uint64_t n, uint32_t L,
                                                        uint32_t a, uint32_t W, uint32_t bias, int* __restrict__ err) {
  const uint64_t i = (uint64_t)blockIdx.x * 256 + threadIdx.x;
  if (i >= n) return;
  uint32_t w[8];
  load_words16(scalars + i * 8, w, 2);
  uint32_t carry = 0, bit = 0;
  for (uint32_t win = 0; win < W; win++) {
    const uint32_t c = win < a ? L + 1 : L, word = bit >> 5, off = bit & 31;
    uint32_t v = w[word] >> off;
    if (off + c > 32 && word + 1 < 8) v |= w[word + 1] << (32 - off);
    v = (v & ((1u << c) - 1u)) + carry;
    uint32_t stored;
    if (win < a) {
      carry = v >> L ? 1u : 0u;
      stored = v + bias - (carry << c);
    } else {
      carry = v >> L;
      stored = (v & ((1u << L) - 1u)) + bias;
    }
    digits[(size_t)win * n + i] = (uint16_t)stored;
    bit += c;
  }
  if (carry | (w[7] >> 29)) atomicOr(err, ERR_NARROW_RANGE);
  uint32_t carry16 = 0;
#pragma unroll
  for (uint32_t win = 0; win < 16; win++) carry16 = (((w[win >> 1] >> (16 * (win & 1))) & 0xffffu) + carry16) >= 32768u ? 1u : 0u;
  if (carry16) atomicOr(err, ERR_SCALAR);
}

template <int SB>
__device__ __forceinline__ void load_short_scalar(const uint8_t* __restrict__ scalars, uint64_t i, uint64_t n, uint32_t* w ) {
  if constexpr (SB >= 16) {
    load_words16(reinterpret_cast<const uint32_t*>(scalars + i * SB), w, SB / 16);
  } else {
    constexpr uint64_t PER = 16 / SB;
    const uint64_t g = i / PER;
    if ((g + 1) * PER <= n) {
      uint4 q = reinterpret_cast<const uint4*>(scalars)[g];
      asm volatile("" : "+v"(q.x), "+v"(q.y), "+v"(q.z), "+v"(q.w));
      const uint32_t k = (uint32_t)(i % PER);
      if constexpr (SB == 8) {
        w[0] = k ? q.z : q.x;
        w[1] = k ? q.w : q.y;
      } else {
        w[0] = k == 0 ? q.x : k == 1 ? q.y : k == 2 ? q.z : q.w;
      }
    } else if constexpr (SB == 8) {
      const uint2 q = reinterpret_cast<const uint2*>(scalars)[i];
      w[0] = q.x;
      w[1] = q.y;
    } else {
      w[0] = reinterpret_cast<const uint32_t*>(scalars)[i];
    }
  }
}

template <int SB>
__global__ void __launch_bounds__(256) k_decompose_short(const uint8_t* __restrict__ scalars, uint16_t* __restrict__ digits, uint64_t n, uint32_t bits, uint32_t L,
                                                         uint32_t W, uint32_t bias, uint32_t top_bias, int* __restrict__ err, uint32_t* __restrict__ top_key_max) {
  constexpr int NW = SB / 4;
  __shared__ uint32_t wmax;
  if (threadIdx.x == 0) wmax = 0;
  __syncthreads();
  const uint64_t i = (uint64_t)blockIdx.x * 256 + threadIdx.x;
  if (i < n) {
    uint32_t w[NW];
    load_short_scalar<SB>(scalars, i, n, w);
    uint32_t excess = 0;
#pragma unroll
    for (int j = 0; j < NW; j++) {
      const uint32_t lo = 32u * j;
      const uint32_t keep = bits <= lo ? 0u : bits >= lo + 32u ? 0xffffffffu : (1u << (bits - lo)) - 1u;
      excess |= w[j] & ~keep;
      w[j] &= keep;
    }
    if (excess) atomicOr(err, ERR_SHORT_WIDTH);
    const uint32_t c = L + 1, mask = (1u << c) - 1u;
    uint32_t carry = 0;
    for (uint32_t win = 0; win + 1 < W; win++) {
      const uint32_t v = (w[0] & mask) + carry;
      carry = v >> L ? 1u : 0u;
      digits[(size_t)win * n + i] = (uint16_t)(v + bias - (carry << c));
#pragma unroll
      for (int j = 0; j + 1 < NW; j++) w[j] = (w[j] >> c) | (w[j + 1] << (32u - c));
      w[NW - 1] >>= c;
    }
    const uint32_t top = w[0] + carry;
    digits[(size_t)(W - 1) * n + i] = (uint16_t)(top + top_bias);
    if (top_key_max && top > wmax) atomicMax(&wmax, top);
  }
  __syncthreads();
  if (threadIdx.x == 0 && top_key_max) atomicMax(top_key_max, wmax | KEY_TRACKED | KEY_UNSIGNED);
}

__global__ void __launch_bounds__(256) k_scalars_width(const uint32_t* __restrict__ words, uint64_t nwords, uint32_t wps, uint32_t* __restrict__ out) {
  __shared__ uint32_t wave_max[4];
  const uint32_t tid = threadIdx.x;
  const uint64_t groups = nwords / 4;
  const uint4* v = reinterpret_cast<const uint4*>(words);
  uint32_t m = 0;
  auto see = [&](uint64_t k, uint32_t x) {
    if (x) {
      const uint32_t len = ((uint32_t)k & (wps - 1u)) * 32u + 32u - (uint32_t)__builtin_clz(x);
      m = len > m ? len : m;
    }
  };
  for (uint64_t g = (uint64_t)blockIdx.x * 256 + tid; g < groups; g += (uint64_t)gridDim.x * 256) {
    const uint4 q = v[g];
    see(4 * g, q.x);
    see(4 * g + 1, q.y);
    see(4 * g + 2, q.z);
    see(4 * g + 3, q.w);
  }
  if (blockIdx.x == 0 && tid < (uint32_t)(nwords & 3)) see(4 * groups + tid, words[4 * groups + tid]);
#pragma unroll
  for (int off = 32; off >= 1; off >>= 1) {
    const uint32_t o = (uint32_t)__shfl_xor((int)m, off, 64);
    m = o > m ? o : m;
  }
  if ((tid & 63) == 0) wave_max[tid >> 6] = m;
  __syncthreads();
  if (tid == 0) {
    for (int k = 1; k < 4; k++) m = wave_max[k] > m ? wave_max[k] : m;
    if (m) atomicMax(out, m);
  }
}

template <int NA, int NB_>
__device__ __forceinline__ void mul_words(const uint32_t* a, const uint32_t* b, uint32_t* out) {
#pragma unroll
  for (int k = 0; k < NA + NB_; k++) out[k] = 0;
#pragma unroll
  for (int i = 0; i < NA; i++) {
    uint32_t carry = 0;
#pragma unroll
    for (int j = 0; j < NB_; j++) {
      const uint64_t t = (uint64_t)a[i] * b[j] + out[i + j] + carry;
      out[i + j] = (uint32_t)t;
      carry = (uint32_t)(t >> 32);
    }
    out[i + NB_] = carry;
  }
}

__device__ __forceinline__ uint32_t recode128(const uint32_t* v, uint16_t* __restrict__ digits, size_t stride, size_t col, uint32_t wb,
                                              uint32_t wc) {
  uint32_t carry = 0, bad = 0;
#pragma unroll
  for (uint32_t win = 0; win < 8; win++) {
    const uint32_t limb = (v[win >> 1] >> (16 * (win & 1))) & 0xffffu;
    const uint32_t t = limb + carry;
    carry = (win < 7 && t >= 32768u) ? 1u : 0u;
    if (win >= wb && win < wb + wc) digits[(size_t)(win - wb) * stride + col] = (uint16_t)((t + 32768u) & 0xffffu);
    if (win == 7 && t >= 32768u) bad = 1u;
  }
  return bad;
}

__global__ void __launch_bounds__(256) k_decompose_glv(const uint32_t* __restrict__ scalars, uint16_t* __restrict__ digits, uint64_t n,
                                                       uint32_t wb, uint32_t wc, int* __restrict__ err) {
  uint64_t i = (uint64_t)blockIdx.x * 256 + threadIdx.x;
  if (i >= n) return;
  uint32_t k[8];
  load_words16(scalars + i * 8, k, 2);
  uint32_t prod[17];
  mul_words<8, 9>(k, GlvConsts::MU, prod);
  uint32_t q[5];
#pragma unroll
  for (int j = 0; j < 5; j++) q[j] = prod[12 + j];
  uint32_t ql[9];
  mul_words<5, 4>(q, GlvConsts::LAMBDA, ql);
  uint32_t rem[5];
  {
    uint32_t borrow = 0;
#pragma unroll
    for (int j = 0; j < 5; j++) {
      const uint64_t d = (uint64_t)k[j] - ql[j] - borrow;
      rem[j] = (uint32_t)d;
      borrow = (uint32_t)(d >> 32) & 1u;
    }
  }
  uint32_t sub[5];
  uint32_t borrow = 0;
#pragma unroll
  for (int j = 0; j < 5; j++) {
    const uint64_t d = (uint64_t)rem[j] - (j < 4 ? GlvConsts::LAMBDA[j] : 0u) - borrow;
    sub[j] = (uint32_t)d;
    borrow = (uint32_t)(d >> 32) & 1u;
  }
  if (!borrow) {
#pragma unroll
    for (int j = 0; j < 5; j++) rem[j] = sub[j];
    uint32_t c = 1;
#pragma unroll
    for (int j = 0; j < 5; j++) {
      const uint64_t t = (uint64_t)q[j] + c;
      q[j] = (uint32_t)t;
      c = (uint32_t)(t >> 32);
    }
  }
  uint32_t bad = q[4] | rem[4];
  bad |= recode128(rem, digits, (size_t)2 * n, (size_t)i, wb, wc);
  bad |= recode128(q, digits, (size_t)2 * n, (size_t)(n + i), wb, wc);
  if (bad) atomicOr(err, 2);
}

}
}
```

### webgpu-msm-bls12-377_amd/csrc/kernels/sort.hpp

```cpp
#pragma once
#include "../curves.hpp"
#include "decompose.hpp"

namespace msm377 {
namespace {



template <class F>
__device__ __forceinline__ void for_each_digit(const uint16_t* __restrict__ dg, uint64_t beg, uint64_t end, uint32_t tid, uint32_t nthreads, F f) {
  uint64_t head = beg;
  while (head < end && (((uintptr_t)(dg + head)) & 15)) head++;
  for (uint64_t i = beg + tid; i < head; i += nthreads) f(i, (uint32_t)dg[i]);
  const uint64_t groups = (end - head) / 8;
  const uint4* v = reinterpret_cast<const uint4*>(dg + head);
  for (uint64_t g = tid; g < groups; g += nthreads) {
    const uint4 q = v[g];
    const uint32_t w[4] = {q.x, q.y, q.z, q.w};
#pragma unroll
    for (int k = 0; k < 4; k++) {
      f(head + g * 8 + 2 * k, w[k] & 0xffffu);
      f(head + g * 8 + 2 * k + 1, w[k] >> 16);
    }
  }
  for (uint64_t i = head + groups * 8 + tid; i < end; i += nthreads) f(i, (uint32_t)dg[i]);
}

template <bool UNS = false>
__global__ void __launch_bounds__(1024) k_range_count(const uint16_t* __restrict__ digits, uint32_t* __restrict__ counts ,
                                                      uint64_t n, uint32_t chunks, uint64_t per_chunk, const uint32_t* __restrict__ key_max) {
  __shared__ uint32_t cnt[NRANGE];
  const uint32_t c = blockIdx.x, ws = blockIdx.y, tid = threadIdx.x;
  const uint32_t shift = win_shift(key_max[ws]);
  const bool uns = UNS && (key_max[ws] & KEY_UNSIGNED) != 0;
  if (tid < NRANGE) cnt[tid] = 0;
  __syncthreads();
  const uint64_t beg = (uint64_t)c * per_chunk;
  const uint64_t end = (beg + per_chunk < n) ? beg + per_chunk : n;
  for_each_digit(digits + (size_t)ws * n, beg, end, tid, 1024, [&](uint64_t, uint32_t biased) {
    uint32_t key, sign;
    digit_key(biased, uns, key, sign);
    atomicAdd(&cnt[key_range(key, shift)], 1u);
  });
  __syncthreads();
  if (tid < NRANGE) counts[((size_t)ws * NRANGE + tid) * chunks + c] = cnt[tid];
}

__global__ void __launch_bounds__(NRANGE) k_range_scan(uint32_t* __restrict__ counts, uint32_t* __restrict__ region_base, uint32_t chunks) {
  __shared__ uint32_t part[NRANGE];
  const uint32_t ws = blockIdx.x, r = threadIdx.x;
  uint32_t* cr = counts + ((size_t)ws * NRANGE + r) * chunks;
  uint32_t tot = 0;
  for (uint32_t c = 0; c < chunks; c++) tot += cr[c];
  part[r] = tot;
  __syncthreads();
  for (uint32_t off = 1; off < NRANGE; off <<= 1) {
    const uint32_t v = r >= off ? part[r - off] : 0u;
    __syncthreads();
    part[r] += v;
    __syncthreads();
  }
  const uint32_t base = part[r] - tot;
  region_base[ws * (NRANGE + 1) + r] = base;
  if (r == NRANGE - 1) region_base[ws * (NRANGE + 1) + NRANGE] = part[r];
  uint32_t run = base;
  for (uint32_t c = 0; c < chunks; c++) {
    const uint32_t v = cr[c];
    cr[c] = run;
    run += v;
  }
}

template <class E>
struct ElemOps;
template <>
struct ElemOps<SortElem> {
  static constexpr bool TAGGED = false;
  static __device__ __forceinline__ SortElem make(uint32_t idx, uint32_t sign, uint32_t key, uint32_t, uint32_t) { return SortElem{idx | (sign << 31), key}; }
  static __device__ __forceinline__ SortElem none(uint32_t lo) { return SortElem{0u, lo}; }
  static __device__ __forceinline__ uint32_t bin(SortElem e, uint32_t lo) { return e.key - lo; }
  static __device__ __forceinline__ uint32_t idx_sign(SortElem e) { return e.idx_sign; }
};
template <>
struct ElemOps<SortElem4> {
  static constexpr bool TAGGED = true;
  static __device__ __forceinline__ SortElem4 make(uint32_t idx, uint32_t sign, uint32_t key, uint32_t rg, uint32_t shift) {
    return sort_pack(idx, sign, key - range_first_key(rg, shift));
  }
  static __device__ __forceinline__ SortElem4 none(uint32_t) { return SortElem4{0u}; }
  static __device__ __forceinline__ uint32_t bin(SortElem4 e, uint32_t) { return sort_sub(e); }
  static __device__ __forceinline__ uint32_t idx_sign(SortElem4 e) { return sort_idx_sign(e); }
};

constexpr uint32_t PT_TILE = 8192;
template <class E, bool UNS = false>
__global__ void __launch_bounds__(1024) k_partition_staged(const uint16_t* __restrict__ digits, const uint32_t* __restrict__ counts,
                                                           E* __restrict__ temp, uint64_t n, uint32_t chunks, uint64_t per_chunk,
                                                           const uint32_t* __restrict__ key_max) {
  using Ops = ElemOps<E>;
  __shared__ uint32_t cur[NRANGE];
  __shared__ uint32_t cnt[NRANGE];
  __shared__ uint32_t toff[NRANGE];
  __shared__ uint32_t gdelta[NRANGE];
  __shared__ uint32_t wsum[NRANGE / 64];
  __shared__ E stage[PT_TILE];
  __shared__ uint8_t tag[Ops::TAGGED ? PT_TILE : 1];
  static_assert(NRANGE <= 256, "a range fits the one-byte tag");
  const uint32_t c = blockIdx.x, ws = blockIdx.y, tid = threadIdx.x;
  const uint32_t shift = win_shift(key_max[ws]);
  const bool uns = UNS && (key_max[ws] & KEY_UNSIGNED) != 0;
  if (tid < NRANGE) {
    cur[tid] = counts[((size_t)ws * NRANGE + tid) * chunks + c];
    cnt[tid] = 0;
  }
  __syncthreads();
  const uint64_t beg = (uint64_t)c * per_chunk;
  const uint64_t end = (beg + per_chunk < n) ? beg + per_chunk : n;
  const uint16_t* dg = digits + (size_t)ws * n;
  E* out = temp + (size_t)ws * n;
  for (uint64_t tile0 = beg; tile0 < end; tile0 += PT_TILE) {
    const uint64_t i0 = tile0 + (uint64_t)tid * 8;
    uint32_t d[8];
    uint32_t valid = 0;
    if (i0 + 8 <= end && (((uintptr_t)(dg + i0)) & 15) == 0) {
      const uint4 q = *reinterpret_cast<const uint4*>(dg + i0);
      const uint32_t w[4] = {q.x, q.y, q.z, q.w};
#pragma unroll
      for (int k = 0; k < 4; k++) {
        d[2 * k] = w[k] & 0xffffu;
        d[2 * k + 1] = w[k] >> 16;
      }
      valid = 0xffu;
    } else {
#pragma unroll
      for (int j = 0; j < 8; j++) {
        d[j] = 0;
        if (i0 + j < end) {
          d[j] = dg[i0 + j];
          valid |= 1u << j;
        }
      }
    }
    uint32_t key[8], sign[8], rg[8], rk[8];
#pragma unroll
    for (int j = 0; j < 8; j++) {
      digit_key(d[j], uns, key[j], sign[j]);
      rg[j] = key_range(key[j], shift);
      rk[j] = 0;
      if ((valid >> j) & 1u) rk[j] = atomicAdd(&cnt[rg[j]], 1u);
    }
    __syncthreads();
    uint32_t mine = 0, incl = 0;
    if (tid < NRANGE) {
      mine = cnt[tid];
      incl = mine;
#pragma unroll
      for (int off = 1; off < 64; off <<= 1) {
        const uint32_t v = __shfl_up((int)incl, off, 64);
        if ((tid & 63) >= (uint32_t)off) incl += v;
      }
      if ((tid & 63) == 63) wsum[tid >> 6] = incl;
    }
    __syncthreads();
    if (tid < NRANGE) {
      uint32_t before = 0;
      for (uint32_t w = 0; w < (tid >> 6); w++) before += wsum[w];
      const uint32_t excl = before + incl - mine;
      toff[tid] = excl;
      gdelta[tid] = cur[tid] - excl;
      cur[tid] += mine;
      cnt[tid] = 0;
    }
    __syncthreads();
#pragma unroll
    for (int j = 0; j < 8; j++)
      if ((valid >> j) & 1u) {
        const uint32_t slot = toff[rg[j]] + rk[j];
        stage[slot] = Ops::make((uint32_t)(i0 + j), sign[j], key[j], rg[j], shift);
        if constexpr (Ops::TAGGED) tag[slot] = (uint8_t)rg[j];
      }
    __syncthreads();
    const uint32_t tile_len = (uint32_t)((end - tile0 < PT_TILE) ? end - tile0 : PT_TILE);
    for (uint32_t p = tid; p < tile_len; p += 1024) {
      const E e = stage[p];
      uint32_t range;
      if constexpr (Ops::TAGGED)
        range = tag[p];
      else
        range = key_range(e.key, shift);
      out[gdelta[range] + p] = e;
    }
    __syncthreads();
  }
}

constexpr uint32_t LS_CACHE = 6144;
constexpr uint32_t LS_REG = LS_CACHE / 256;
template <class E>
__global__ void __launch_bounds__(256) k_local_sort_lds(const E* __restrict__ temp, const uint32_t* __restrict__ region_base,
                                                        uint32_t* __restrict__ row_ptr, uint32_t* __restrict__ val_idx, uint64_t n,
                                                        const uint32_t* __restrict__ key_max, uint32_t NR, uint32_t NBK) {
  using Ops = ElemOps<E>;
  constexpr uint32_t NBINS = KRANGE + 1;
  static_assert(NBINS <= 256, "one bin per thread");
  __shared__ uint32_t bins[NBINS];
  __shared__ uint32_t part[256];
  __shared__ uint32_t sorted[LS_CACHE];
  const uint32_t RPW = NBK + 2;
  const uint32_t r = blockIdx.x, ws = blockIdx.y, tid = threadIdx.x;
  const uint32_t shift = key_max ? win_shift(key_max[ws]) : 0u;
  const uint32_t KR = KRANGE >> shift;
  const uint32_t lo = r * KR;
  const bool last = shift == 0 && r == NR - 1;
  const uint32_t nb = KR + (last ? 1u : 0u);
  const uint32_t rbeg = region_base[ws * (NR + 1) + r], rend = region_base[ws * (NR + 1) + r + 1];
  const uint32_t len = rend - rbeg;
  const bool cached = len <= LS_CACHE;
  const E* in = temp + (size_t)ws * n + rbeg;
  if (tid < NBINS) bins[tid] = 0;
  __syncthreads();
  E e[LS_REG];
  if (cached) {
#pragma unroll
    for (uint32_t u = 0; u < LS_REG; u++) {
      const uint32_t i = u * 256 + tid;
      e[u] = Ops::none(lo);
      if (i < len) e[u] = in[i];
    }
#pragma unroll
    for (uint32_t u = 0; u < LS_REG; u++)
      if (u * 256 + tid < len) atomicAdd(&bins[Ops::bin(e[u], lo)], 1u);
  } else {
    for (uint32_t i0 = 0; i0 < len; i0 += 2048) {
      E f[8];
#pragma unroll
      for (int u = 0; u < 8; u++) {
        const uint32_t i = i0 + u * 256 + tid;
        f[u] = Ops::none(lo);
        if (i < len) f[u] = in[i];
      }
#pragma unroll
      for (int u = 0; u < 8; u++)
        if (i0 + u * 256 + tid < len) atomicAdd(&bins[Ops::bin(f[u], lo)], 1u);
    }
  }
  __syncthreads();
  const uint32_t own = tid < nb ? bins[tid] : 0u;
  part[tid] = own;
  __syncthreads();
  for (uint32_t off = 1; off < 256; off <<= 1) {
    const uint32_t v = tid >= off ? part[tid - off] : 0u;
    __syncthreads();
    part[tid] += v;
    __syncthreads();
  }
  uint32_t* rp = row_ptr + (size_t)ws * RPW + lo;
  const uint32_t start = rbeg + part[tid] - own;
  __syncthreads();
  if (tid < nb) {
    bins[tid] = start;
    rp[tid] = start;
  }
  if (tid == 0 && last) rp[nb] = rend;
  if (shift) {
    const uint32_t covered = NR * KR, total = region_base[ws * (NR + 1) + NR];
    const uint32_t per_block = (RPW - covered + NR - 1) / NR;
    uint32_t* rp_w = row_ptr + (size_t)ws * RPW;
    for (uint32_t j = tid; j < per_block; j += 256) {
      const uint32_t idx = covered + r * per_block + j;
      if (idx < RPW) rp_w[idx] = total;
    }
  }
  __syncthreads();
  uint32_t* vi = val_idx + (size_t)ws * n;
  if (cached) {
#pragma unroll
    for (uint32_t u = 0; u < LS_REG; u++)
      if (u * 256 + tid < len) sorted[atomicAdd(&bins[Ops::bin(e[u], lo)], 1u) - rbeg] = Ops::idx_sign(e[u]);
    __syncthreads();
    for (uint32_t i = tid; i < len; i += 256) vi[rbeg + i] = sorted[i];
  } else {
    for (uint32_t i0 = 0; i0 < len; i0 += 2048) {
      E f[8];
#pragma unroll
      for (int u = 0; u < 8; u++) {
        const uint32_t i = i0 + u * 256 + tid;
        f[u] = Ops::none(lo);
        if (i < len) f[u] = in[i];
      }
#pragma unroll
      for (int u = 0; u < 8; u++) {
        const uint32_t i = i0 + u * 256 + tid;
        if (i < len) vi[atomicAdd(&bins[Ops::bin(f[u], lo)], 1u)] = Ops::idx_sign(f[u]);
      }
    }
  }
}

__global__ void __launch_bounds__(1024) k_small_sort(const uint16_t* __restrict__ digits, uint32_t* __restrict__ row_ptr, uint32_t* __restrict__ val_idx,
                                                     uint32_t n, uint32_t L) {
  __shared__ uint32_t bins[SMALL_BINS_MAX + 1];
  __shared__ uint32_t part[1024];
  const uint32_t ws = blockIdx.x, tid = threadIdx.x;
  const uint32_t half = 1u << L, nbins = half + 1;
  const uint16_t* dg = digits + (size_t)ws * n;
  for (uint32_t b = tid; b <= nbins; b += 1024) bins[b] = 0;
  __syncthreads();
  for (uint32_t i = tid; i < n; i += 1024) {
    const int d = (int)dg[i] - (int)half;
    atomicAdd(&bins[d < 0 ? -d : d], 1u);
  }
  __syncthreads();
  const uint32_t per = (nbins + 1023) / 1024;
  uint32_t local = 0;
  for (uint32_t k = 0; k < per; k++) {
    const uint32_t b = tid * per + k;
    if (b < nbins) local += bins[b];
  }
  part[tid] = local;
  __syncthreads();
  for (uint32_t off = 1; off < 1024; off <<= 1) {
    const uint32_t v = tid >= off ? part[tid - off] : 0u;
    __syncthreads();
    part[tid] += v;
    __syncthreads();
  }
  uint32_t run = part[tid] - local;
  uint32_t* rp = row_ptr + (size_t)ws * (half + 2);
  for (uint32_t k = 0; k < per; k++) {
    const uint32_t b = tid * per + k;
    if (b < nbins) {
      const uint32_t cnt = bins[b];
      bins[b] = run;
      rp[b] = run;
      run += cnt;
    }
  }
  if (tid == 0) rp[nbins] = n;
  __syncthreads();
  uint32_t* vi = val_idx + (size_t)ws * n;
  for (uint32_t i = tid; i < n; i += 1024) {
    const int d = (int)dg[i] - (int)half;
    vi[atomicAdd(&bins[d < 0 ? -d : d], 1u)] = i | (d < 0 ? 0x80000000u : 0u);
  }
}

}
}
```

### webgpu-msm-bls12-377_amd/csrc/sequencer.hip

```cpp
#include "sequencer.hpp"

#include <hip/hip_runtime.h>
#include <string.h>

#include <algorithm>
#include <atomic>
#include <chrono>
#include <functional>
#include <thread>
#include <type_traits>
#include <vector>

#include "context.hpp"
#include "host_tail.hpp"
#include "validate_host.hpp"
#include "kernels/accumulate.hpp"
#include "kernels/batch_mul.hpp"
#include "kernels/convert.hpp"
#include "kernels/decompose.hpp"
#include "kernels/generate.hpp"
#include "kernels/reduce.hpp"
#include "kernels/sort.hpp"
#include "kernels/validate.hpp"
#include "kernels/import.hpp"
#include "kernels/wide.hpp"

bool WideBuffers::ensure(uint64_t n) {
  using namespace msm377;
  if (cap >= n) return true;
  release();
  if (hipMalloc((void**)&digits, (size_t)WIDE_WINDOWS * n * 4) == hipSuccess && hipMalloc((void**)&temp, (size_t)WIDE_WINDOWS * n * sizeof(SortElem)) == hipSuccess &&
      hipMalloc((void**)&counts, WC_WORDS * 4) == hipSuccess) {
    cap = n;
    return true;
  }
  release();
  (void)hipGetLastError();
  return false;
}

namespace msm377 {
namespace eng {

bool hip_ok(msm377_ctx* ctx, int hip_error, const char* what) {
  const hipError_t e = (hipError_t)hip_error;
  if (e == hipSuccess) return true;
  if (ctx) ctx->err = std::string(what) + ": " + hipGetErrorString(e);
  return false;
}

namespace {

void note_fallback(msm377_ctx* ctx, uint32_t mask) {
  ctx->fallback_count++;
  ctx->fallback_mask = mask;
}
#define HIP_TRY(ctx, call)                            \
  do {                                                \
    if (!msm377::eng::hip_ok((ctx), (int)(call), #call)) return MSM377_EHIP; \
  } while (0)

struct HipFail {
  hipError_t e = hipSuccess;
  const char* what = "";
  int record(msm377_ctx* ctx, int rc) const {
    hip_ok(ctx, e, what);
    return rc;
  }
};
int h2d_staged(msm377_ctx* ctx, void* d_dst, const uint8_t* src, size_t bytes, size_t stage_off, HipFail* fail = nullptr) {
  using msm377::eng::reserve_host_staging;
#define H2D_TRY(call)                \
  do {                               \
    const hipError_t e_ = (call);    \
    if (e_ != hipSuccess) {          \
      if (fail) *fail = {e_, #call}; \
      else hip_ok(ctx, e_, #call);   \
      return MSM377_EHIP;            \
    }                                \
  } while (0)
  constexpr int NT_MAX = 8;
  constexpr int NT = 4;
  constexpr size_t SMALL = 8u << 20, PIECE = 4u << 20;
  if (bytes < SMALL) {
    H2D_TRY(hipMemcpy(d_dst, src, bytes, hipMemcpyHostToDevice));
    return MSM377_OK;
  }
  if (!ctx->h_stage && reserve_host_staging(ctx) != MSM377_OK) {
    (void)hipGetLastError();
    H2D_TRY(hipMemcpy(d_dst, src, bytes, hipMemcpyHostToDevice));
    return MSM377_OK;
  }
  size_t npieces = (bytes + PIECE - 1) / PIECE;
  npieces = (npieces + NT - 1) / NT * NT;
  const size_t piece = ((bytes + npieces - 1) / npieces + 4095) & ~(size_t)4095;
  uint8_t* stage = ctx->h_stage + stage_off;
  hipError_t errs[NT_MAX + 1];
  std::thread workers[NT_MAX];
  const int device = ctx->device;
  std::atomic<size_t> next{0};
  auto copy_pieces = [&, device](int t) {
    hipError_t e = hipSetDevice(device);
    for (;;) {
      const size_t c = next.fetch_add(1, std::memory_order_relaxed);
      const size_t off = c * piece;
      if (c >= npieces || off >= bytes || e != hipSuccess) break;
      const size_t len = (bytes - off < piece) ? bytes - off : piece;
      memcpy(stage + off, src + off, len);
      e = hipMemcpyAsync((uint8_t*)d_dst + off, stage + off, len, hipMemcpyHostToDevice, ctx->copy_stream[t]);
    }
    if (e == hipSuccess) e = hipStreamSynchronize(ctx->copy_stream[t]);
    errs[t] = e;
  };
  for (int t = 0; t <= NT; t++) errs[t] = hipSuccess;
  for (int t = 0; t < NT; t++) workers[t] = std::thread([&copy_pieces, t] { copy_pieces(t); });
  copy_pieces(NT);
  for (int t = 0; t < NT; t++) workers[t].join();
  for (int t = 0; t <= NT; t++) H2D_TRY(errs[t]);
  return MSM377_OK;
#undef H2D_TRY
}

void identity_wire(uint8_t out[96]) {
  memset(out, 0, 96);
  out[48] = 1;
}

struct StageTimer {
  msm377_ctx* c;
  int s;
  hipStream_t st;
  bool on() const { return c->timing == 1 || (c->timing == 2 && s == MSM377_STAGE_ACC_KERNEL); }
  StageTimer(msm377_ctx* ctx, int stage, hipStream_t stream) : c(ctx), s(stage), st(stream) {
    if (on()) (void)hipEventRecord(c->ev[s][0], st);
  }
  ~StageTimer() {
    if (on()) (void)hipEventRecord(c->ev[s][1], st);
  }
};

template <class CV>
int convert_bases(msm377_ctx* ctx, const uint32_t* d_raw, uint64_t n, uint64_t first = 0, bool clear_err = true) {
  if (n == 0) return MSM377_OK;
  if (ctx->timing == 1) (void)hipEventRecord(ctx->ev[MSM377_STAGE_CONVERT][0], ctx->stream2);
  if (clear_err) hipLaunchKernelGGL(k_clear_words, dim3(1), dim3(256), 0, ctx->stream2, (uint32_t*)(ctx->d_err + 2), 1u, (uint32_t*)nullptr, 0u);
  hipLaunchKernelGGL(k_convert_bases<CV>, dim3((unsigned)((n + 255) / 256)), dim3(256), 0, ctx->stream2, d_raw, ctx->d_bases + first * CV::REC_WORDS, n,
                     ctx->d_err + 2);
  HIP_TRY(ctx, hipGetLastError());
  if (ctx->timing == 1) (void)hipEventRecord(ctx->ev[MSM377_STAGE_CONVERT][1], ctx->stream2);
  HIP_TRY(ctx, hipEventRecord(ctx->bases_ready, ctx->stream2));
  return MSM377_OK;
}

int affine_convert_begin(msm377_ctx* ctx, const uint32_t* d_raw, uint64_t n, const uint32_t* prev_window_records = nullptr, uint32_t doublings = 0,
                         bool clear_err = true) {
  if (n == 0) return MSM377_OK;
  const uint32_t nblk = affine_blocks(n);
  if (ctx->timing == 1) (void)hipEventRecord(ctx->ev[MSM377_STAGE_CONVERT][0], ctx->stream2);
  __atomic_store_n(ctx->h_aff_flag, 0u, __ATOMIC_RELEASE);
  if (clear_err) hipLaunchKernelGGL(k_clear_words, dim3(1), dim3(256), 0, ctx->stream2, (uint32_t*)(ctx->d_err + 2), 1u, (uint32_t*)nullptr, 0u);
  if (prev_window_records)
    hipLaunchKernelGGL(k_affine_up<AffDoublingSource>, dim3(nblk), dim3(AFF_THREADS), 0, ctx->stream2, AffDoublingSource{prev_window_records, doublings}, n,
                       ctx->d_aff_stash, ctx->d_aff_trees, ctx->dm_aff_prod, ctx->dm_aff_flag, ctx->d_aff_count, ctx->d_err + 2, ctx->conv_wave_prio);
  else
    hipLaunchKernelGGL(k_affine_up<AffWireSource>, dim3(nblk), dim3(AFF_THREADS), 0, ctx->stream2, AffWireSource{d_raw}, n, ctx->d_aff_stash, ctx->d_aff_trees,
                       ctx->dm_aff_prod, ctx->dm_aff_flag, ctx->d_aff_count, ctx->d_err + 2, ctx->conv_wave_prio);
  HIP_TRY(ctx, hipGetLastError());
  HIP_TRY(ctx, hipEventRecord(ctx->aff_up_done, ctx->stream2));
  if (ctx->tail_threads > 1 && nblk >= 32) ctx->tail_pool.prewake(ctx->aff_prewake_us, std::min(ctx->tail_threads, TailPool::WORKERS + 1) - 1);
  return MSM377_OK;
}

int affine_convert_finish(msm377_ctx* ctx, uint32_t* d_records_out, uint64_t n, bool behind_sort = false) {
  if (n == 0) return MSM377_OK;
  const uint32_t nblk = affine_blocks(n);
  const auto t0 = std::chrono::steady_clock::now();
  for (uint32_t spins = 0; __atomic_load_n(ctx->h_aff_flag, __ATOMIC_ACQUIRE) != nblk; spins++) {
    __builtin_ia32_pause();
    if ((spins & 0xfff) == 0xfff && std::chrono::steady_clock::now() - t0 > std::chrono::milliseconds(20)) {
      HIP_TRY(ctx, hipEventSynchronize(ctx->aff_up_done));
      break;
    }
  }
  if (__atomic_load_n(ctx->h_aff_flag, __ATOMIC_ACQUIRE) != nblk) {
    ctx->err = "batched affine conversion: the block products did not arrive";
    return MSM377_EHIP;
  }
  {
    const int inv_rc = invert_block_products_mt(ctx, 0, nblk);
    ctx->tail_pool.disarm();
    if (inv_rc) return inv_rc;
  }
  hipLaunchKernelGGL(k_affine_down, dim3(nblk), dim3(AFF_THREADS), 0, ctx->stream2, n, ctx->d_aff_stash, ctx->d_aff_trees, ctx->dm_aff_inv, d_records_out, ctx->conv_wave_prio);
  HIP_TRY(ctx, hipGetLastError());
  if (ctx->timing == 1) (void)hipEventRecord(ctx->ev[MSM377_STAGE_CONVERT][1], ctx->stream2);
  HIP_TRY(ctx, hipEventRecord(ctx->bases_ready, ctx->stream2));
  return MSM377_OK;
}

uint32_t auto_seg(const msm377_ctx* ctx, uint64_t entries, bool glv) {
  const uint32_t forced = glv ? ctx->seg_glv : ctx->seg_plain;
  if (forced) return forced;
  const uint64_t s = ((entries >> 18) + 7) & ~7ull;
  return (uint32_t)std::min<uint64_t>(std::max<uint64_t>(s, SEG_MIN), SEG_MAX);
}


struct Phase {
  bool clear_err = true;
  bool front = true;
  bool into = false;
  bool back = true;
  bool zc_out = false;
  uint64_t base_first = 0;
  const uint32_t* table = nullptr;
  uint64_t table_stride = 0;
  uint32_t cbits = MSM377_WINDOW_BITS;
  uint32_t bucket_log = MSM377_WINDOW_BITS - 1;
  bool wide = false;
  bool even = false;
  const uint32_t* bases_override = nullptr;
  uint32_t short_bytes = 0, short_bits = 0;
};

void launch_decompose_short(hipStream_t st, const void* d_scalars, uint16_t* digits, uint64_t n, uint32_t sbytes, uint32_t bits, uint32_t L, uint32_t W, uint32_t bias,
                            uint32_t top_bias, int* d_err, uint32_t* top_key_max) {
  const dim3 grid((unsigned)((n + 255) / 256)), block(256);
  const uint8_t* sc = (const uint8_t*)d_scalars;
  switch (sbytes) {
    case 4: hipLaunchKernelGGL(k_decompose_short<4>, grid, block, 0, st, sc, digits, n, bits, L, W, bias, top_bias, d_err, top_key_max); break;
    case 8: hipLaunchKernelGGL(k_decompose_short<8>, grid, block, 0, st, sc, digits, n, bits, L, W, bias, top_bias, d_err, top_key_max); break;
    case 16: hipLaunchKernelGGL(k_decompose_short<16>, grid, block, 0, st, sc, digits, n, bits, L, W, bias, top_bias, d_err, top_key_max); break;
    default: hipLaunchKernelGGL(k_decompose_short<32>, grid, block, 0, st, sc, digits, n, bits, L, W, bias, top_bias, d_err, top_key_max); break;
  }
}

template <class CV, class BP = CV>
int enqueue_windows(msm377_ctx* ctx, const uint32_t* d_scalars, uint64_t n_scalars, uint32_t wb, uint32_t wc, int slot, bool glv = false,
                    const Phase& ph = Phase()) {
  const uint64_t n = glv ? 2 * n_scalars : n_scalars;
  hipStream_t st = ctx->stream;
  int* d_err = ctx->d_err + slot;
  uint32_t* d_partials = ctx->d_partials + (size_t)slot * SLOT_WORDS;
  StageLayout& layout = ctx->stage;
  layout.valid = false;
  if (ph.clear_err && !ph.front) hipLaunchKernelGGL(k_clear_words, dim3(1), dim3(256), 0, st, (uint32_t*)d_err, 1u, (uint32_t*)nullptr, 0u);
  ctx->zc_active = ph.zc_out && ph.back && ctx->zc_out && slot == 0 && !ph.table;
  if (ctx->zc_active) ctx->out_seq++;
  const uint32_t L = ph.bucket_log, NB = 1u << L;
  const bool wide = ph.wide;
  const bool narrow = !wide && ph.cbits != MSM377_WINDOW_BITS;
  const uint64_t entries = (wide ? (uint64_t)WIDE_WINDOWS : (uint64_t)wc) * n;
  static_assert((uint64_t)NARROW_EVEN_WINDOWS * SMALL_SORT_MAX / NARROW_SEG + NARROW_EVEN_WINDOWS * (1u << NARROW_LOG) <= (uint64_t)MSM377_NUM_WINDOWS * 32768,
                "narrow work items fit the work-item buffer");
  const uint32_t SEG = (narrow && !ctx->seg_plain) ? (ctx->narrow_seg ? ctx->narrow_seg : (n > 8192 ? 16u : 12u)) : auto_seg(ctx, entries, glv);
  uint16_t* digits = ctx->d_digits;
  uint32_t* range_counts = ctx->d_range_counts;
  uint32_t* region_base = ctx->d_region_base;
  SortElem* sort_temp = ctx->d_sort_temp;
  uint32_t* row_ptr = ctx->d_row_ptr;
  uint32_t* val_idx = ctx->d_val_idx;
  uint32_t* buckets = ctx->d_buckets;
  uint32_t* row_ovf_base = ctx->d_row_ovf_base;
  uint32_t* split_rows = ctx->d_split_rows;
  WorkItem* work = ctx->d_work;
  uint32_t* ovf = ctx->d_ovf;
  const uint32_t* records = ctx->resident.valid() ? ctx->resident.bases : ctx->d_bases;
  const uint32_t* bases = ph.table ? ph.table : ph.bases_override ? ph.bases_override : records + ph.base_first * BP::REC_WORDS;
  uint32_t* meta_block = ctx->d_work_meta;
  uint32_t* key_max = meta_block + (2 * SEG_BINS + 4);
  if (ph.front) {
    hipLaunchKernelGGL(k_clear_words, dim3(1), dim3(256), 0, st, meta_block, META_BLOCK_WORDS, (uint32_t*)d_err, ph.clear_err ? 1u : 0u);
    uint32_t* top_key_max = (!glv && !ph.even && wb + wc == MSM377_NUM_WINDOWS) ? key_max + (wc - 1) : nullptr;
    const uint64_t max_items = (uint64_t)wc * NB + entries / SEG;
    const bool quad_acc = std::is_same<BP, CV>::value && std::is_same<CV, TeDev>::value && narrow && !ph.table && max_items <= ctx->narrow_quad_items;
    {
      StageTimer t(ctx, MSM377_STAGE_DECOMPOSE, st);
      layout.info = msm377_stage_info{};
      layout.info.slots = wc;
      layout.info.bucket_log = L;
      layout.info.columns = entries / wc;
      layout.info.digit_bytes = wide ? 4u : 2u;
      layout.info.row_ptr_len = NB + 2;
      layout.info.bucket_records = NB;
      layout.info.form = CV::FORM_ID;
      layout.info.table_stride = ph.table_stride;
      layout.info.geometry_reruns = ctx->geometry_reruns;
      layout.d_digits = wide ? (const void*)ctx->wide.digits : (const void*)digits;
      layout.d_key_max = (wide || narrow) ? nullptr : key_max;
      static_assert(MAX_WINDOW_SLOTS <= MSM377_STAGE_MAX_SLOTS, "a stage layout names every window slot");
      uint32_t bias = 1u << (MSM377_WINDOW_BITS - 1);
      if (ph.short_bytes) {
        bias = narrow ? NB : 32768u;
        const uint32_t top_bias = narrow ? NB : 0u;
        launch_decompose_short(st, d_scalars, digits, n, ph.short_bytes, ph.short_bits, L, wc, bias, top_bias, d_err, narrow ? nullptr : key_max + (wc - 1));
        for (uint32_t s = 0; s < wc; s++) layout.info.bias[s] = s + 1 < wc ? bias : top_bias;
        layout.info.key_unsigned[wc - 1] = narrow ? 0u : 1u;
      } else if (wide) {
        bias = 1u << WIDE_LOG;
        hipLaunchKernelGGL(k_decompose_wide, dim3((unsigned)((n + 255) / 256)), dim3(256), 0, st, d_scalars, ctx->wide.digits, n, d_err);
      } else if (narrow) {
        bias = 1u << L;
        hipLaunchKernelGGL(k_decompose_geom, dim3((unsigned)((n + 255) / 256)), dim3(256), 0, st, d_scalars, digits, n, L, NARROW_EVEN_SIGNED, wc, bias, d_err);
      } else if (glv)
        hipLaunchKernelGGL(k_decompose_glv, dim3((unsigned)((n_scalars + 255) / 256)), dim3(256), 0, st, d_scalars, digits, n_scalars, wb, wc, d_err);
      else
        hipLaunchKernelGGL(k_decompose, dim3((unsigned)((n + 255) / 256)), dim3(256), 0, st, d_scalars, digits, n, wb, wc, d_err, top_key_max, ph.even ? 1u : 0u);
      if (!ph.short_bytes)
        for (uint32_t s = 0; s < wc; s++) layout.info.bias[s] = bias;
      HIP_TRY(ctx, hipGetLastError());
    }

    if (wide) {
      StageTimer t(ctx, MSM377_STAGE_SORT, st);
      uint32_t* wc = ctx->wide.counts;
      ctx->last_sort_elem = sort_elem_bytes(entries, true);
      hipLaunchKernelGGL(k_wide_count, dim3(WS_CHUNKS, WIDE_WINDOWS), dim3(1024), 0, st, (const uint32_t*)ctx->wide.digits, wc, n);
      hipLaunchKernelGGL(k_wide_sums, dim3(WIDE_NRANGE / 256, WIDE_WINDOWS), dim3(256), 0, st, wc);
      hipLaunchKernelGGL(k_wide_scan, dim3(1), dim3(1024), 0, st, wc, region_base);
      hipLaunchKernelGGL(k_wide_offsets1, dim3(WIDE_WINDOWS), dim3(WS_COARSE), 0, st, wc, n);
      hipLaunchKernelGGL(k_wide_part1, dim3(WS_CHUNKS, WIDE_WINDOWS), dim3(1024), 0, st, (const uint32_t*)ctx->wide.digits, (const uint32_t*)wc, sort_temp, n, (uint32_t)ph.table_stride);
      hipLaunchKernelGGL(k_wide_part2, dim3(WS_COARSE, WIDE_WINDOWS), dim3(1024), 0, st, (const SortElem*)sort_temp, (const uint32_t*)wc, ctx->wide.temp);
      hipLaunchKernelGGL(k_local_sort_lds<SortElem>, dim3(WIDE_NRANGE, 1), dim3(256), 0, st, (const SortElem*)ctx->wide.temp, region_base, row_ptr, val_idx, entries,
                         (const uint32_t*)nullptr, WIDE_NRANGE, NB);
      HIP_TRY(ctx, hipGetLastError());
    } else if (narrow) {
      StageTimer t(ctx, MSM377_STAGE_SORT, st);
      ctx->last_sort_elem = 0;
      hipLaunchKernelGGL(k_small_sort, dim3(wc), dim3(1024), 0, st, digits, row_ptr, val_idx, (uint32_t)n, L);
      HIP_TRY(ctx, hipGetLastError());
    } else {
      StageTimer t(ctx, MSM377_STAGE_SORT, st);
      uint32_t chunks = MAX_SORT_BLOCKS / wc;
      const uint64_t want = (n + 4095) / 4096;
      if (chunks > want) chunks = (uint32_t)(want ? want : 1);
      const uint64_t per_chunk = (n + chunks - 1) / chunks;
      if (ph.short_bytes)
        hipLaunchKernelGGL(k_range_count<true>, dim3(chunks, wc), dim3(1024), 0, st, digits, range_counts, n, chunks, per_chunk, key_max);
      else
        hipLaunchKernelGGL(k_range_count<false>, dim3(chunks, wc), dim3(1024), 0, st, digits, range_counts, n, chunks, per_chunk, key_max);
      HIP_TRY(ctx, hipGetLastError());
      hipLaunchKernelGGL(k_range_scan, dim3(wc), dim3(NRANGE), 0, st, range_counts, region_base, chunks);
      HIP_TRY(ctx, hipGetLastError());
      const bool packed = ctx->sort_elem == 4 && sort_elem_bytes(n, false) == 4;
      ctx->last_sort_elem = packed ? 4u : 8u;
      auto partition_and_sort = [&](auto* temp) {
        using E = std::remove_pointer_t<decltype(temp)>;
        if (ph.short_bytes)
          hipLaunchKernelGGL((k_partition_staged<E, true>), dim3(chunks, wc), dim3(1024), 0, st, digits, range_counts, temp, n, chunks, per_chunk, key_max);
        else
          hipLaunchKernelGGL((k_partition_staged<E, false>), dim3(chunks, wc), dim3(1024), 0, st, digits, range_counts, temp, n, chunks, per_chunk, key_max);
        const hipError_t e = hipGetLastError();
        if (e != hipSuccess) return e;
        hipLaunchKernelGGL(k_local_sort_lds<E>, dim3(NRANGE, wc), dim3(256), 0, st, (const E*)temp, region_base, row_ptr, val_idx, n, key_max, NRANGE, NB);
        return hipGetLastError();
      };
      HIP_TRY(ctx, packed ? partition_and_sort(reinterpret_cast<SortElem4*>(sort_temp)) : partition_and_sort(sort_temp));
    }

    {
      StageTimer t(ctx, MSM377_STAGE_ACCUMULATE, st);
      const uint32_t rows = wc * NB;
      uint32_t* meta = meta_block;
      uint32_t* work_hist = meta;
      uint32_t* cursor = meta + SEG_BINS;
      uint32_t* total = meta + 2 * SEG_BINS;
      uint32_t* counters = meta + 2 * SEG_BINS + 1;
      hipLaunchKernelGGL(k_work_hist, dim3((rows + 1023) / 1024), dim3(1024), 0, st, row_ptr, L, rows, SEG, work_hist, row_ovf_base, counters, split_rows);
      HIP_TRY(ctx, hipGetLastError());
      hipLaunchKernelGGL(k_work_scatter, dim3((rows + 1023) / 1024), dim3(1024), 0, st, row_ptr, L, rows, SEG, (const uint32_t*)work_hist, cursor, total, work);
      HIP_TRY(ctx, hipGetLastError());
      if (ctx->before_accumulate) {
        std::function<int()> f;
        f.swap(ctx->before_accumulate);
        const int hook_rc = f();
        if (hook_rc) return hook_rc;
      }
      HIP_TRY(ctx, hipStreamWaitEvent(st, ctx->bases_ready, 0));
      ctx->last_products = BP::MADD_PRODUCTS;
      {
        StageTimer tk(ctx, MSM377_STAGE_ACC_KERNEL, st);
        const dim3 grid((unsigned)((max_items + 255) / 256));
        bool launched = false;
        if constexpr (std::is_same<BP, CV>::value && std::is_same<CV, TeDev>::value) {
          if (quad_acc) {
            hipLaunchKernelGGL(k_accumulate_quad<CV>, dim3((unsigned)((4 * max_items + 255) / 256)), dim3(256), 0, st, row_ptr, val_idx, bases, buckets, n, work, total,
                               row_ovf_base, ovf, SEG, d_err, ctx->d_err + 2, ph.into ? 1u : 0u, L);
            launched = true;
          }
        }
        if (launched) {
        } else if constexpr (!std::is_same<BP, CV>::value)
          hipLaunchKernelGGL((k_accumulate<CV, 2, BP>), grid, dim3(256), 0, st, row_ptr, val_idx, bases, buckets, n, work, total, row_ovf_base, ovf, SEG, d_err,
                             ctx->d_err + 2, ph.into ? 1u : 0u, ph.table_stride, L);
        else
          hipLaunchKernelGGL((k_accumulate<CV, 2>), grid, dim3(256), 0, st, row_ptr, val_idx, bases, buckets, n, work, total, row_ovf_base, ovf, SEG, d_err,
                             ctx->d_err + 2, ph.into ? 1u : 0u, ph.table_stride, L);
      }
      HIP_TRY(ctx, hipGetLastError());
      ctx->acc_seq++;
      static_assert(CV::HAS_QUAD, "every curve policy has the quad-cooperative addition");
      if (ph.short_bytes) {
        hipLaunchKernelGGL(k_fold_long_rows<CV>, dim3(FOLD_BLOCKS), dim3(FOLD_THREADS), 0, st, row_ptr, row_ovf_base, ovf, SEG, d_err, L, wc - 1);
        HIP_TRY(ctx, hipGetLastError());
      }
      hipLaunchKernelGGL(k_merge_split_rows_quad<CV>, dim3(std::min<uint32_t>((rows + 63) / 64, 1024u)), dim3(256), 0, st, row_ptr, buckets, counters, split_rows, row_ovf_base, ovf, SEG, d_err, L,
                         ctx->dm_out_flag + ACC_FLAG_WORD, ctx->acc_seq);
      HIP_TRY(ctx, hipGetLastError());
    }
  }
  if (!ph.back) return MSM377_OK;
  if (ctx->capture) {
    HIP_TRY(ctx, hipMemcpyAsync(ctx->d_buckets_snap, buckets, (size_t)wc * CV::BKT_WORDS * NB * 4, hipMemcpyDeviceToDevice, st));
  }
  const uint32_t wc_out = ph.table ? 1u : wc;
  const uint32_t pp = wide ? WIDE_POINTS : (uint32_t)MSM377_G1_PARTIAL_POINTS;
  {
    StageTimer t(ctx, MSM377_STAGE_REDUCE, st);
    if (ph.table) {
      for (uint32_t m = wc; m > 1;) {
        const uint32_t half = (m + 1) / 2, count = m - half;
        hipLaunchKernelGGL(k_fold_windows<CV>, dim3(count * NB / 256), dim3(256), 0, st, buckets, L, half, count, d_err);
        HIP_TRY(ctx, hipGetLastError());
        m = half;
      }
    }
    const uint32_t levels = L;
    uint32_t coop_from = 0;
    for (coop_from = 0; coop_from < levels && 4ull * (coop_from + 1) * (NB >> (coop_from + 1)) * wc_out > ctx->coop_threads; coop_from++) {
      }
    const uint32_t tail_from = CV::HAS_QUAD ? std::min(wide ? levels - 8 : narrow ? ctx->narrow_tail_from : ctx->tail_from, levels) : levels;
    uint32_t r = 0;
    if (ctx->reduce_columns) {
      while (r < tail_from) {
        const uint32_t k = std::min(tail_from - r, COLUMN_LEVELS_MAX);
        const uint32_t threads = (r + 1) * (NB >> (r + 1));
        hipLaunchKernelGGL(k_tree_columns<CV>, dim3((threads + 255) / 256, wc_out), dim3(256), 0, st, buckets, L, r, k, coop_from, threads, d_err);
        HIP_TRY(ctx, hipGetLastError());
        r += k;
      }
    }
    for (; r < tail_from; r++) {
      const uint32_t ops = (r + 1) * (NB >> (r + 1));
      bool done = false;
      if constexpr (CV::HAS_QUAD) {
        if (r >= coop_from) {
          hipLaunchKernelGGL(k_tree_step_quad<CV>, dim3((4 * ops + 255) / 256, wc_out), dim3(256), 0, st, buckets, L, r, ops, d_err);
          done = true;
        }
      }
      if (!done) hipLaunchKernelGGL(k_tree_step<CV>, dim3((ops + 255) / 256, wc_out), dim3(256), 0, st, buckets, L, r, ops, d_err);
      HIP_TRY(ctx, hipGetLastError());
    }
    if constexpr (CV::HAS_QUAD) {
      if (tail_from < levels) {
        const size_t lds_bytes = (size_t)(NB >> tail_from) * CV::PT_WORDS * 4;
        if (ctx->tail_lds && lds_bytes > 64 * 1024 && lds_bytes <= TAIL_LDS_BYTES_MAX)
          HIP_TRY(ctx, hipFuncSetAttribute(reinterpret_cast<const void*>(&k_reduce_tail_lds<CV>), hipFuncAttributeMaxDynamicSharedMemorySize, (int)TAIL_LDS_BYTES_MAX));
        if (ctx->tail_lds && lds_bytes <= TAIL_LDS_BYTES_MAX)
          hipLaunchKernelGGL(k_reduce_tail_lds<CV>, dim3(tail_from + 1, wc_out), dim3(TAIL_THREADS), lds_bytes, st, buckets, L, tail_from, d_err);
        else
          hipLaunchKernelGGL(k_reduce_tail<CV>, dim3(tail_from + 1, wc_out), dim3(TAIL_THREADS), 0, st, buckets, L, tail_from, d_err);
        HIP_TRY(ctx, hipGetLastError());
      }
    }
    if (ctx->zc_active)
      hipLaunchKernelGGL(k_gather_partials<CV>, dim3((wc_out * pp * 4 + 63) / 64), dim3(64), 0, st, buckets, d_partials, wc_out, L, ctx->dm_partials,
                         ctx->dm_out_flag, ctx->d_out_count, (const int*)d_err, ctx->out_seq, pp);
    else
      hipLaunchKernelGGL(k_gather_partials<CV>, dim3((wc_out * pp * 4 + 63) / 64), dim3(64), 0, st, buckets, d_partials, wc_out, L, (uint32_t*)nullptr,
                         (uint32_t*)nullptr, (uint32_t*)nullptr, (const int*)nullptr, 0u, pp);
    HIP_TRY(ctx, hipGetLastError());
  }
  if (!ctx->zc_active) {
    HIP_TRY(ctx, hipMemcpyAsync(ctx->h_partials + (size_t)slot * SLOT_WORDS, d_partials, (size_t)wc_out * pp * CV::OUT_WORDS * 4,
                                 hipMemcpyDeviceToHost, st));
    HIP_TRY(ctx, hipMemcpyAsync(ctx->h_err + slot, d_err, sizeof(int), hipMemcpyDeviceToHost, st));
  }
  HIP_TRY(ctx, hipEventRecord(ctx->done_ev[slot], st));
  ctx->last_n = n;
  ctx->last_wc = wc;
  ctx->last_geom_windows = wc;
  ctx->last_geom_log = L;
  ctx->last_glv = glv;
  ctx->last_form = CV::FORM_ID;
  layout.valid = ctx->capture && ph.front && !ph.into && wb == 0 && CV::FORM_ID >= 0;
  return MSM377_OK;
}

int wait_zero_copy_out(msm377_ctx* ctx) {
  const auto t0 = std::chrono::steady_clock::now();
  for (uint32_t spins = 0; __atomic_load_n(&ctx->h_out_flag[0], __ATOMIC_ACQUIRE) != ctx->out_seq; spins++) {
    __builtin_ia32_pause();
    if ((spins & 0xfff) == 0xfff && std::chrono::steady_clock::now() - t0 > std::chrono::milliseconds(50)) {
      HIP_TRY(ctx, hipEventSynchronize(ctx->done_ev[0]));
      break;
    }
  }
  if (__atomic_load_n(&ctx->h_out_flag[0], __ATOMIC_ACQUIRE) != ctx->out_seq) {
    ctx->err = "zero-copy output: the window records did not arrive";
    return MSM377_EHIP;
  }
  ctx->h_err[0] = (int)__atomic_load_n(&ctx->h_out_flag[1], __ATOMIC_RELAXED);
  return MSM377_OK;
}

int finish_windows(msm377_ctx* ctx, int slot) {
  if (ctx->zc_active && slot == 0) {
    const int rc = wait_zero_copy_out(ctx);
    if (rc) return rc;
    if (ctx->timing) HIP_TRY(ctx, hipEventSynchronize(ctx->done_ev[slot]));
  } else {
    HIP_TRY(ctx, hipEventSynchronize(ctx->done_ev[slot]));
  }
  if (ctx->timing) {
    for (int s = 0; s < MSM377_NUM_STAGES; s++) {
      if (s == MSM377_STAGE_TAIL) continue;
      if (ctx->timing == 2 && s != MSM377_STAGE_ACC_KERNEL) {
        ctx->stage_ms[s] = 0.0;
        continue;
      }
      float ms = 0.f;
      ctx->stage_ms[s] = hipEventElapsedTime(&ms, ctx->ev[s][0], ctx->ev[s][1]) == hipSuccess ? ms : 0.0;
    }
    (void)hipGetLastError();
  }
  if (ctx->h_err[slot] & ERR_SCALAR) {
    ctx->err = "a scalar overflows the signed 16-bit window recode (final carry)";
    return MSM377_ESCALAR;
  }
  return MSM377_OK;
}

template <class CV>
int run_windows(msm377_ctx* ctx, const uint32_t* d_scalars, uint64_t n, uint32_t wb, uint32_t wc, bool glv = false) {
  int rc = enqueue_windows<CV>(ctx, d_scalars, n, wb, wc, 0, glv);
  if (rc) return rc;
  return finish_windows(ctx, 0);
}

inline bool use_glv(const msm377_ctx* ctx, uint64_t) { return ctx->glv_mode == 1; }

int convert_bases_g1(msm377_ctx* ctx, const uint32_t* d_raw, uint64_t n, bool glv) {
  if (!glv) return convert_bases<G1Dev>(ctx, d_raw, n);
  if (n == 0) return MSM377_OK;
  if (ctx->timing == 1) (void)hipEventRecord(ctx->ev[MSM377_STAGE_CONVERT][0], ctx->stream2);
  hipLaunchKernelGGL(k_clear_words, dim3(1), dim3(256), 0, ctx->stream2, (uint32_t*)(ctx->d_err + 2), 1u, (uint32_t*)nullptr, 0u);
  hipLaunchKernelGGL(k_convert_bases_glv, dim3((unsigned)((n + 255) / 256)), dim3(256), 0, ctx->stream2, d_raw, ctx->d_bases, n);
  HIP_TRY(ctx, hipGetLastError());
  if (ctx->timing == 1) (void)hipEventRecord(ctx->ev[MSM377_STAGE_CONVERT][1], ctx->stream2);
  HIP_TRY(ctx, hipEventRecord(ctx->bases_ready, ctx->stream2));
  return MSM377_OK;
}

enum TableForm { TABLE_XYZZ = 0, TABLE_XYZZ_GLV = 1, TABLE_TE = 2, TABLE_TE_AFFINE = 3, TABLE_TE_PRECOMP = 4 };
inline bool form_is_te(int form) { return form == TABLE_TE || form == TABLE_TE_AFFINE || form == TABLE_TE_PRECOMP; }
constexpr int RC_TE_FALLBACK = 1;

inline int resident_form(const msm377_ctx* ctx, uint64_t n) {
  return (ctx->resident.form == TABLE_XYZZ_GLV && n != ctx->resident.n) ? TABLE_XYZZ : ctx->resident.form;
}
inline bool wide_table(const ResidentBases& r) { return r.form == TABLE_TE_PRECOMP && r.windows == WIDE_WINDOWS; }
inline int weierstrass_form(const msm377_ctx* ctx, uint64_t n) { return use_glv(ctx, n) ? TABLE_XYZZ_GLV : TABLE_XYZZ; }
inline int pick_form(const msm377_ctx* ctx, uint64_t n) { return ctx->g1_form == 1 ? TABLE_TE : weierstrass_form(ctx, n); }

int convert_table(msm377_ctx* ctx, const uint32_t* d_raw, uint64_t n, int form) {
  if (form == TABLE_TE) return convert_bases<TeDev>(ctx, d_raw, n);
  if (form == TABLE_TE_AFFINE) {
    const int rc = affine_convert_begin(ctx, d_raw, n);
    return rc ? rc : affine_convert_finish(ctx, ctx->d_bases, n);
  }
  return convert_bases_g1(ctx, d_raw, n, form == TABLE_XYZZ_GLV);
}

void time_tail(msm377_ctx* ctx, std::chrono::steady_clock::time_point t0) {
  ctx->stage_ms[MSM377_STAGE_TAIL] = std::chrono::duration<double, std::milli>(std::chrono::steady_clock::now() - t0).count();
}

struct TailArm {
  msm377_ctx* c;
  bool armed = false;
  explicit TailArm(msm377_ctx* ctx) : c(ctx) {}
  void arm() {
    if (armed || c->tail_threads <= 1 || c->tail_spin_us <= 0) return;
    armed = true;
    c->tail_pool.prewake(c->tail_spin_us, std::min(c->tail_threads, TailPool::WORKERS + 1) - 1);
  }
  void at_start(uint64_t n) {
    if (n <= (1ull << 17)) arm();
  }
  void after_accumulation() {
    if (armed || c->tail_threads <= 1 || c->tail_spin_us <= 0) return;
    const auto t0 = std::chrono::steady_clock::now();
    for (uint32_t spins = 0; __atomic_load_n(&c->h_out_flag[ACC_FLAG_WORD], __ATOMIC_ACQUIRE) != c->acc_seq; spins++) {
      __builtin_ia32_pause();
      if ((spins & 0xfff) == 0xfff && std::chrono::steady_clock::now() - t0 > std::chrono::milliseconds(100)) return;
    }
    arm();
  }
  ~TailArm() { c->tail_pool.disarm(); }
};

int g1_table_msm(msm377_ctx* ctx, const uint32_t* d_scalars, uint64_t n, int form, uint8_t out_xy[96]) {
  TailArm arm(ctx);
  arm.at_start(n);
  if (form_is_te(form)) {
    Phase ph;
    if (form == TABLE_TE_PRECOMP) {
      ph.table = ctx->resident.table;
      ph.table_stride = ctx->resident.n;
    }
    bool narrow = form != TABLE_TE_PRECOMP && n <= ctx->narrow_max_points && n <= SMALL_SORT_MAX && ctx->capture != 1;
    bool wide = form == TABLE_TE_PRECOMP && wide_table(ctx->resident);
    bool table0 = false;
    bool even = ctx->even_windows && form != TABLE_TE_PRECOMP && ctx->capture != 1;
    for (;;) {
      uint32_t windows = MSM377_NUM_WINDOWS;
      int cbits = MSM377_WINDOW_BITS, planes = MSM377_WINDOW_BITS - 1, short_from = 0;
      ph.cbits = MSM377_WINDOW_BITS;
      ph.bucket_log = MSM377_WINDOW_BITS - 1;
      if (wide) {
        ph.wide = true;
        ph.cbits = WIDE_BITS;
        ph.bucket_log = WIDE_LOG;
        windows = 1;
        cbits = WIDE_BITS;
        planes = WIDE_LOG;
      } else if (narrow) {
        ph.cbits = NARROW_EVEN_BITS;
        ph.bucket_log = NARROW_LOG;
        windows = NARROW_EVEN_WINDOWS;
        cbits = NARROW_EVEN_BITS;
        planes = NARROW_LOG;
        short_from = NARROW_EVEN_SIGNED;
      }
      ph.even = even && !wide && !table0;
      if (ph.even && !narrow) short_from = EVEN_FROM;
      ph.zc_out = true;
      int rc = form == TABLE_TE ? enqueue_windows<TeDev>(ctx, d_scalars, n, 0, windows, 0, false, ph)
                                : enqueue_windows<TeDev, TeAffBase>(ctx, d_scalars, n, 0, windows, 0, false, ph);
      if (rc) return rc;
      arm.after_accumulation();
      if (ctx->zc_active) {
        rc = wait_zero_copy_out(ctx);
        if (rc) return rc;
      } else {
        HIP_TRY(ctx, hipEventSynchronize(ctx->done_ev[0]));
      }
      if (narrow && (ctx->h_err[0] & ERR_NARROW_RANGE) && !(ctx->h_err[0] & ERR_SCALAR)) {
        narrow = false;
        even = false;
        ctx->geometry_reruns++;
        continue;
      }
      if (ph.even && (ctx->h_err[0] & ERR_NARROW_RANGE) && !(ctx->h_err[0] & ERR_SCALAR)) {
        even = false;
        ctx->geometry_reruns++;
        continue;
      }
      if (wide && (ctx->h_err[0] & ERR_NARROW_RANGE) && !(ctx->h_err[0] & ERR_SCALAR)) {
        wide = false;
        table0 = true;
        ctx->geometry_reruns++;
        ph.wide = false;
        ph.table = nullptr;
        ph.table_stride = 0;
        ph.bases_override = ctx->resident.table;
        continue;
      }
      if (ctx->h_err[0] & ERR_TE_ANY) {
        note_fallback(ctx, (uint32_t)(ctx->h_err[0] & ERR_TE_ANY));
        return RC_TE_FALLBACK;
// ... 1297 lines not shown
```

Baseline: 2.353.

## Fold range count into decompose and scan/work-hist into partition and local sort

Adds a fused decompose+count kernel that builds per-chunk range histograms while writing digits, so the separate range-count pass over the digits is skipped. The range prefix scan moves into the partition kernel: each block recomputes totals from all chunk counts. The work histogram and split-row bookkeeping move into the local sort kernel, which removes two more launches. The count layout is transposed to chunk-major and stored next to the meta block so a single parallel clear zeroes both. The cost is redundant scan work in every partition block and extra atomics.

```diff
diff --git a/webgpu-msm-bls12-377_amd/csrc/capi.hip b/webgpu-msm-bls12-377_amd/csrc/capi.hip
--- a/webgpu-msm-bls12-377_amd/csrc/capi.hip
+++ b/webgpu-msm-bls12-377_amd/csrc/capi.hip
@@ -75,6 +75,7 @@
   if (const char* e = getenv("MSM377_REDUCE_COLUMNS")) ctx->reduce_columns = atoi(e) != 0;
   if (const char* e = getenv("MSM377_EVEN_WINDOWS")) ctx->even_windows = atoi(e) != 0;
   if (const char* e = getenv("MSM377_SORT_ELEM")) ctx->sort_elem = atoi(e) == 4 ? 4u : 8u;
+  if (const char* e = getenv("MSM377_FRONT_FOLD")) ctx->front_fold = atoi(e) != 0;
   if (const char* e = getenv("MSM377_TWIN_BATCH")) ctx->twin_batches = atoi(e) != 0;
   if (const char* e = getenv("MSM377_BASE_CHECKS")) ctx->base_checks = check_flags_normal((uint32_t)strtoul(e, nullptr, 0));
   if (const char* e = getenv("MSM377_TAIL_FROM")) ctx->tail_from = (uint32_t)std::min(std::max(atoi(e), 1), (int)TREE_LEVELS);
@@ -91,7 +92,6 @@
   dalloc((void**)&ctx->d_bases, 2 * cap * G1_REC_WORDS * 4);
   const uint64_t wcap = std::max<uint64_t>((uint64_t)MSM377_NUM_WINDOWS * cap, (uint64_t)NARROW_EVEN_WINDOWS * std::min<uint64_t>(cap, SMALL_SORT_MAX));
   dalloc((void**)&ctx->d_digits, wcap * 2);
-  dalloc((void**)&ctx->d_range_counts, (size_t)NRANGE * MAX_SORT_BLOCKS * 4);
   dalloc((void**)&ctx->d_region_base, (size_t)MSM377_NUM_WINDOWS * (NRANGE + 1) * 4);
   dalloc((void**)&ctx->d_sort_temp, cap * MSM377_NUM_WINDOWS * sizeof(SortElem));
   dalloc((void**)&ctx->d_row_ptr, (size_t)MSM377_NUM_WINDOWS * RP * 4);
@@ -100,7 +100,8 @@
   dalloc((void**)&ctx->d_partials, (size_t)2 * SLOT_WORDS * 4);
   const uint64_t extra_items = std::max<uint64_t>((uint64_t)MSM377_NUM_WINDOWS * cap / SEG_MIN, (uint64_t)NARROW_EVEN_WINDOWS * std::min<uint64_t>(cap, SMALL_SORT_MAX) / NARROW_SEG) + 2;
   dalloc((void**)&ctx->d_work, ((size_t)MSM377_NUM_WINDOWS * NB + extra_items) * sizeof(WorkItem));
-  dalloc((void**)&ctx->d_work_meta, (size_t)META_BLOCK_WORDS * 4);
+  dalloc((void**)&ctx->d_work_meta, ((size_t)META_BLOCK_WORDS + (size_t)NRANGE * MAX_SORT_BLOCKS) * 4);
+  ctx->d_range_counts = ctx->d_work_meta ? ctx->d_work_meta + META_BLOCK_WORDS : nullptr;
   dalloc((void**)&ctx->d_row_ovf_base, (size_t)MSM377_NUM_WINDOWS * NB * 4);
   dalloc((void**)&ctx->d_split_rows, (size_t)MSM377_NUM_WINDOWS * NB * 4);
   dalloc((void**)&ctx->d_ovf, (size_t)extra_items * BKT_WORDS * 4);
@@ -149,7 +150,7 @@
     msm377_ctx_destroy(ctx->twin);
     ctx->twin = nullptr;
   }
-  void* bufs[] = {ctx->d_raw_points, ctx->d_raw_scalars, ctx->d_bases, ctx->d_digits, ctx->d_range_counts, ctx->d_region_base, ctx->d_sort_temp,
+  void* bufs[] = {ctx->d_raw_points, ctx->d_raw_scalars, ctx->d_bases, ctx->d_digits, ctx->d_region_base, ctx->d_sort_temp,
                   ctx->d_row_ptr, ctx->d_val_idx, ctx->d_buckets, ctx->d_buckets_snap, ctx->d_partials, ctx->d_work, ctx->d_work_meta, ctx->d_row_ovf_base, ctx->d_split_rows, ctx->d_ovf, ctx->d_err, ctx->d_aff_stash, ctx->d_aff_trees, ctx->d_aff_count, ctx->d_out_count, ctx->resident.table, ctx->d_native, ctx->d_inf_mask,
                   ctx->bm.table, ctx->bm.stash, ctx->bm.trees, ctx->bm.block_prod, ctx->bm.block_inv, ctx->bm.row_bases, ctx->bm.base_wire};
   for (void* p : bufs)
diff --git a/webgpu-msm-bls12-377_amd/csrc/common.hpp b/webgpu-msm-bls12-377_amd/csrc/common.hpp
--- a/webgpu-msm-bls12-377_amd/csrc/common.hpp
+++ b/webgpu-msm-bls12-377_amd/csrc/common.hpp
@@ -64,6 +64,22 @@
   uint32_t row;
   uint32_t seg;
 };
+struct RowSplit {
+  uint32_t nseg, seglen, lastlen;
+};
+MSM_HD RowSplit row_split(uint32_t len, uint32_t SEG) {
+  RowSplit r;
+  if (len <= SEG) {
+    r.nseg = 1;
+    r.seglen = r.lastlen = len;
+    return r;
+  }
+  const uint32_t parts = (len + SEG - 1) / SEG;
+  r.seglen = (len + parts - 1) / parts;
+  r.nseg = (len + r.seglen - 1) / r.seglen;
+  r.lastlen = len - (r.nseg - 1) * r.seglen;
+  return r;
+}
 constexpr uint32_t META_BLOCK_WORDS = 2 * SEG_BINS + 4 + MSM377_NUM_WINDOWS;
 constexpr size_t SLOT_WORDS = (size_t)MAX_WINDOW_SLOTS * MSM377_G1_PARTIAL_POINTS * MSM377_G1_POINT_WORDS;
 
diff --git a/webgpu-msm-bls12-377_amd/csrc/context.hpp b/webgpu-msm-bls12-377_amd/csrc/context.hpp
--- a/webgpu-msm-bls12-377_amd/csrc/context.hpp
+++ b/webgpu-msm-bls12-377_amd/csrc/context.hpp
@@ -159,6 +159,7 @@
   bool tail_lds = true;
   bool even_windows = true;
   uint32_t sort_elem = 8;
+  bool front_fold = true;
   bool ed_equal_windows_once = false;
   uint32_t acc_seq = 0;
   msm377_ctx* twin = nullptr;
diff --git a/webgpu-msm-bls12-377_amd/csrc/kernels/accumulate.hpp b/webgpu-msm-bls12-377_amd/csrc/kernels/accumulate.hpp
--- a/webgpu-msm-bls12-377_amd/csrc/kernels/accumulate.hpp
+++ b/webgpu-msm-bls12-377_amd/csrc/kernels/accumulate.hpp
@@ -15,22 +15,6 @@
   return row_ptr[at + 1] - row_ptr[at];
 }
 
-struct RowSplit {
-  uint32_t nseg, seglen, lastlen;
-};
-__device__ __forceinline__ RowSplit row_split(uint32_t len, uint32_t SEG) {
-  RowSplit r;
-  if (len <= SEG) {
-    r.nseg = 1;
-    r.seglen = r.lastlen = len;
-    return r;
-  }
-  const uint32_t parts = (len + SEG - 1) / SEG;
-  r.seglen = (len + parts - 1) / parts;
-  r.nseg = (len + r.seglen - 1) / r.seglen;
-  r.lastlen = len - (r.nseg - 1) * r.seglen;
-  return r;
-}
 
 __global__ void __launch_bounds__(1024) k_work_hist(const uint32_t* __restrict__ row_ptr, uint32_t L, uint32_t rows, uint32_t SEG, uint32_t* __restrict__ work_hist,
                                                    uint32_t* __restrict__ row_ovf_base, uint32_t* __restrict__ counters ,
diff --git a/webgpu-msm-bls12-377_amd/csrc/kernels/convert.hpp b/webgpu-msm-bls12-377_amd/csrc/kernels/convert.hpp
--- a/webgpu-msm-bls12-377_amd/csrc/kernels/convert.hpp
+++ b/webgpu-msm-bls12-377_amd/csrc/kernels/convert.hpp
@@ -6,8 +6,9 @@
 
 
 __global__ void __launch_bounds__(256) k_clear_words(uint32_t* __restrict__ a, uint32_t na, uint32_t* __restrict__ b, uint32_t nb) {
-  for (uint32_t i = threadIdx.x; i < na; i += 256) a[i] = 0;
-  for (uint32_t i = threadIdx.x; i < nb; i += 256) b[i] = 0;
+  const uint32_t first = blockIdx.x * 256 + threadIdx.x, step = gridDim.x * 256;
+  for (uint32_t i = first; i < na; i += step) a[i] = 0;
+  for (uint32_t i = first; i < nb; i += step) b[i] = 0;
 }
 
 template <class CV>
diff --git a/webgpu-msm-bls12-377_amd/csrc/kernels/decompose.hpp b/webgpu-msm-bls12-377_amd/csrc/kernels/decompose.hpp
--- a/webgpu-msm-bls12-377_amd/csrc/kernels/decompose.hpp
+++ b/webgpu-msm-bls12-377_amd/csrc/kernels/decompose.hpp
@@ -24,6 +24,27 @@
   return s == 0 ? (key >= NB ? NRANGE - 1 : key / KRANGE) : key >> (7 - s);
 }
 
+__device__ __forceinline__ int recode_even(const uint32_t* w, uint32_t* biased ) {
+  uint32_t carry = 0;
+  uint32_t carry16 = 0;
+#pragma unroll
+  for (uint32_t win = 0; win < 16; win++) {
+    const uint32_t limb = (w[win >> 1] >> (16 * (win & 1))) & 0xffffu;
+    carry16 = limb + carry16 >= 32768u ? 1u : 0u;
+    if (win < EVEN_FROM) {
+      const uint32_t v = limb + carry;
+      carry = v >= 32768u ? 1u : 0u;
+      biased[win] = (v + 32768u) & 0xffffu;
+    } else {
+      const uint32_t raw = win == 13 ? (w[6] >> 16) & 0x7fffu : win == 14 ? (w[6] >> 31) | ((w[7] & 0x3fffu) << 1) : (w[7] >> 14) & 0x7fffu;
+      const uint32_t v = raw + carry;
+      carry = v >> 15;
+      biased[win] = (v & 0x7fffu) + 32768u;
+    }
+  }
+  return ((carry | (w[7] >> 29)) ? ERR_NARROW_RANGE : 0) | (carry16 ? ERR_SCALAR : 0);
+}
+
 __global__ void __launch_bounds__(256) k_decompose(const uint32_t* __restrict__ scalars, uint16_t* __restrict__ digits, uint64_t n,
                                                    uint32_t wb, uint32_t wc, int* __restrict__ err, uint32_t* __restrict__ top_key_max, uint32_t even) {
   __shared__ uint32_t wmax;
@@ -35,26 +56,13 @@
     load_words16(scalars + i * 8, w, 2);
     uint32_t carry = 0;
     if (even) {
-      uint32_t carry16 = 0;
-#pragma unroll
-      for (uint32_t win = 0; win < 16; win++) {
-        const uint32_t limb = (w[win >> 1] >> (16 * (win & 1))) & 0xffffu;
-        carry16 = limb + carry16 >= 32768u ? 1u : 0u;
-        uint32_t biased;
-        if (win < EVEN_FROM) {
-          const uint32_t v = limb + carry;
-          carry = v >= 32768u ? 1u : 0u;
-          biased = (v + 32768u) & 0xffffu;
-        } else {
-          const uint32_t raw = win == 13 ? (w[6] >> 16) & 0x7fffu : win == 14 ? (w[6] >> 31) | ((w[7] & 0x3fffu) << 1) : (w[7] >> 14) & 0x7fffu;
-          const uint32_t v = raw + carry;
-          carry = v >> 15;
-          biased = (v & 0x7fffu) + 32768u;
-        }
-        if (win >= wb && win < wb + wc) digits[(size_t)(win - wb) * n + i] = (uint16_t)biased;
-      }
-      if (carry | (w[7] >> 29)) atomicOr(err, ERR_NARROW_RANGE);
-      if (carry16) atomicOr(err, ERR_SCALAR);
+      uint32_t biased[16];
+      const int flags = recode_even(w, biased);
+#pragma unroll
+      for (uint32_t win = 0; win < 16; win++)
+        if (win >= wb && win < wb + wc) digits[(size_t)(win - wb) * n + i] = (uint16_t)biased[win];
+      if (flags & ERR_NARROW_RANGE) atomicOr(err, ERR_NARROW_RANGE);
+      if (flags & ERR_SCALAR) atomicOr(err, ERR_SCALAR);
     } else {
 #pragma unroll
       for (uint32_t win = 0; win < 16; win++) {
@@ -76,6 +84,46 @@
   }
   __syncthreads();
   if (threadIdx.x == 0 && top_key_max && wmax > *top_key_max) atomicMax(top_key_max, wmax);
+}
+
+constexpr uint32_t DC_THREADS = 512, DC_PER_THREAD = 4, DC_SCALARS = DC_THREADS * DC_PER_THREAD;
+__global__ void __launch_bounds__(DC_THREADS) k_decompose_count(const uint32_t* __restrict__ scalars, uint16_t* __restrict__ digits,
+                                                                uint32_t* __restrict__ counts , uint64_t n, uint32_t wb, uint32_t wc,
+                                                                uint32_t chunks, uint64_t per_chunk, int* __restrict__ err) {
+  __shared__ uint32_t cnt[MSM377_NUM_WINDOWS * NRANGE];
+  const uint32_t c = blockIdx.y, tid = threadIdx.x;
+  for (uint32_t j = tid; j < wc * NRANGE; j += DC_THREADS) cnt[j] = 0;
+  __syncthreads();
+  const uint64_t cbeg = (uint64_t)c * per_chunk;
+  const uint64_t cend = (cbeg + per_chunk < n) ? cbeg + per_chunk : n;
+  const uint64_t beg = cbeg + (uint64_t)blockIdx.x * DC_SCALARS;
+  uint32_t w[DC_PER_THREAD][8];
+#pragma unroll
+  for (uint32_t u = 0; u < DC_PER_THREAD; u++) {
+    const uint64_t i = beg + u * DC_THREADS + tid;
+    if (i < cend) load_words16(scalars + i * 8, w[u], 2);
+  }
+  int flags = 0;
+#pragma unroll
+  for (uint32_t u = 0; u < DC_PER_THREAD; u++) {
+    const uint64_t i = beg + u * DC_THREADS + tid;
+    if (i < cend) {
+      uint32_t biased[16];
+      flags |= recode_even(w[u], biased);
+#pragma unroll
+      for (uint32_t win = 0; win < 16; win++)
+        if (win >= wb && win < wb + wc) {
+          digits[(size_t)(win - wb) * n + i] = (uint16_t)biased[win];
+          uint32_t key, sign;
+          digit_key(biased[win], key, sign);
+          atomicAdd(&cnt[(win - wb) * NRANGE + key_range(key, 0)], 1u);
+        }
+    }
+  }
+  if (flags) atomicOr(err, flags);
+  __syncthreads();
+  for (uint32_t j = tid; j < wc * NRANGE; j += DC_THREADS)
+    if (const uint32_t v = cnt[j]) atomicAdd(&counts[((size_t)(j / NRANGE) * chunks + c) * NRANGE + j % NRANGE], v);
 }
 
 
diff --git a/webgpu-msm-bls12-377_amd/csrc/kernels/sort.hpp b/webgpu-msm-bls12-377_amd/csrc/kernels/sort.hpp
--- a/webgpu-msm-bls12-377_amd/csrc/kernels/sort.hpp
+++ b/webgpu-msm-bls12-377_amd/csrc/kernels/sort.hpp
@@ -43,15 +43,15 @@
     atomicAdd(&cnt[key_range(key, shift)], 1u);
   });
   __syncthreads();
-  if (tid < NRANGE) counts[((size_t)ws * NRANGE + tid) * chunks + c] = cnt[tid];
+  if (tid < NRANGE) counts[((size_t)ws * chunks + c) * NRANGE + tid] = cnt[tid];
 }
 
 __global__ void __launch_bounds__(NRANGE) k_range_scan(uint32_t* __restrict__ counts, uint32_t* __restrict__ region_base, uint32_t chunks) {
   __shared__ uint32_t part[NRANGE];
   const uint32_t ws = blockIdx.x, r = threadIdx.x;
-  uint32_t* cr = counts + ((size_t)ws * NRANGE + r) * chunks;
+  uint32_t* cr = counts + (size_t)ws * chunks * NRANGE + r;
   uint32_t tot = 0;
-  for (uint32_t c = 0; c < chunks; c++) tot += cr[c];
+  for (uint32_t c = 0; c < chunks; c++) tot += cr[c * NRANGE];
   part[r] = tot;
   __syncthreads();
   for (uint32_t off = 1; off < NRANGE; off <<= 1) {
@@ -65,8 +65,8 @@
   if (r == NRANGE - 1) region_base[ws * (NRANGE + 1) + NRANGE] = part[r];
   uint32_t run = base;
   for (uint32_t c = 0; c < chunks; c++) {
-    const uint32_t v = cr[c];
-    cr[c] = run;
+    const uint32_t v = cr[c * NRANGE];
+    cr[c * NRANGE] = run;
     run += v;
   }
 }
@@ -93,10 +93,10 @@
 };
 
 constexpr uint32_t PT_TILE = 8192;
-template <class E, bool UNS = false>
+template <class E, bool UNS = false, bool SCAN = false>
 __global__ void __launch_bounds__(1024) k_partition_staged(const uint16_t* __restrict__ digits, const uint32_t* __restrict__ counts,
                                                            E* __restrict__ temp, uint64_t n, uint32_t chunks, uint64_t per_chunk,
-                                                           const uint32_t* __restrict__ key_max) {
+                                                           const uint32_t* __restrict__ key_max, uint32_t* __restrict__ region_base) {
   using Ops = ElemOps<E>;
   __shared__ uint32_t cur[NRANGE];
   __shared__ uint32_t cnt[NRANGE];
@@ -109,8 +109,43 @@
   const uint32_t c = blockIdx.x, ws = blockIdx.y, tid = threadIdx.x;
   const uint32_t shift = win_shift(key_max[ws]);
   const bool uns = UNS && (key_max[ws] & KEY_UNSIGNED) != 0;
-  if (tid < NRANGE) {
-    cur[tid] = counts[((size_t)ws * NRANGE + tid) * chunks + c];
+  if constexpr (SCAN) {
+    if (tid < NRANGE) toff[tid] = gdelta[tid] = 0;
+    __syncthreads();
+    const uint32_t* cw = counts + (size_t)ws * chunks * NRANGE;
+    for (uint32_t j = tid; j < NRANGE * chunks; j += 1024) {
+      const uint32_t v = cw[j], r = j % NRANGE;
+      if (v) {
+        atomicAdd(&toff[r], v);
+        if (j / NRANGE < c) atomicAdd(&gdelta[r], v);
+      }
+    }
+    __syncthreads();
+    uint32_t mine = 0, incl = 0;
+    if (tid < NRANGE) {
+      mine = toff[tid];
+      incl = mine;
+#pragma unroll
+      for (int off = 1; off < 64; off <<= 1) {
+        const uint32_t v = __shfl_up((int)incl, off, 64);
+        if ((tid & 63) >= (uint32_t)off) incl += v;
+      }
+      if ((tid & 63) == 63) wsum[tid >> 6] = incl;
+    }
+    __syncthreads();
+    if (tid < NRANGE) {
+      uint32_t before = 0;
+      for (uint32_t w = 0; w < (tid >> 6); w++) before += wsum[w];
+      const uint32_t base = before + incl - mine;
+      cur[tid] = base + gdelta[tid];
+      cnt[tid] = 0;
+      if (c == 0) {
+        region_base[ws * (NRANGE + 1) + tid] = base;
+        if (tid == NRANGE - 1) region_base[ws * (NRANGE + 1) + NRANGE] = base + mine;
+      }
+    }
+  } else if (tid < NRANGE) {
+    cur[tid] = counts[((size_t)ws * chunks + c) * NRANGE + tid];
     cnt[tid] = 0;
   }
   __syncthreads();
@@ -194,18 +229,24 @@
   }
 }
 
-constexpr uint32_t LS_CACHE = 6144;
-constexpr uint32_t LS_REG = LS_CACHE / 256;
 template <class E>
+constexpr uint32_t LS_CACHE = sizeof(E) == 4 ? 8192 : 6144;
+template <class E, bool WH = false>
 __global__ void __launch_bounds__(256) k_local_sort_lds(const E* __restrict__ temp, const uint32_t* __restrict__ region_base,
                                                         uint32_t* __restrict__ row_ptr, uint32_t* __restrict__ val_idx, uint64_t n,
-                                                        const uint32_t* __restrict__ key_max, uint32_t NR, uint32_t NBK) {
+                                                        const uint32_t* __restrict__ key_max, uint32_t NR, uint32_t NBK, uint32_t SEG,
+                                                        uint32_t* __restrict__ work_hist, uint32_t* __restrict__ row_ovf_base,
+                                                        uint32_t* __restrict__ counters ,
+                                                        uint32_t* __restrict__ split_rows) {
   using Ops = ElemOps<E>;
+  constexpr uint32_t CACHE = LS_CACHE<E>, LS_REG = CACHE / 256;
   constexpr uint32_t NBINS = KRANGE + 1;
   static_assert(NBINS <= 256, "one bin per thread");
   __shared__ uint32_t bins[NBINS];
   __shared__ uint32_t part[256];
-  __shared__ uint32_t sorted[LS_CACHE];
+  __shared__ uint32_t sorted[CACHE];
+  __shared__ uint32_t lh[WH ? SEG_BINS : 1];
+  __shared__ uint32_t blk[4];
   const uint32_t RPW = NBK + 2;
   const uint32_t r = blockIdx.x, ws = blockIdx.y, tid = threadIdx.x;
   const uint32_t shift = key_max ? win_shift(key_max[ws]) : 0u;
@@ -215,9 +256,13 @@
   const uint32_t nb = KR + (last ? 1u : 0u);
   const uint32_t rbeg = region_base[ws * (NR + 1) + r], rend = region_base[ws * (NR + 1) + r + 1];
   const uint32_t len = rend - rbeg;
-  const bool cached = len <= LS_CACHE;
+  const bool cached = len <= CACHE;
   const E* in = temp + (size_t)ws * n + rbeg;
   if (tid < NBINS) bins[tid] = 0;
+  if constexpr (WH) {
+    if (tid < SEG_BINS) lh[tid] = 0;
+    if (tid < 2) blk[tid] = 0;
+  }
   __syncthreads();
   E e[LS_REG];
   if (cached) {
@@ -270,8 +315,38 @@
       const uint32_t idx = covered + r * per_block + j;
       if (idx < RPW) rp_w[idx] = total;
     }
-  }
-  __syncthreads();
+    if constexpr (WH) {
+      const uint32_t first = covered + r * per_block, end = first + per_block < NBK + 1 ? first + per_block : NBK + 1;
+      if (tid == 0 && first < end) atomicAdd(&lh[0], end - first);
+    }
+  }
+  RowSplit sp = {1, 0, 0};
+  uint32_t my_split = 0, my_ovf = 0;
+  const uint32_t row = ws * NBK + lo + tid - 1;
+  if constexpr (WH) {
+    if (tid < nb && lo + tid >= 1) {
+      sp = row_split(own, SEG);
+      atomicAdd(&lh[sp.lastlen], 1u);
+      if (sp.nseg > 1) {
+        atomicAdd(&lh[sp.seglen], sp.nseg - 1);
+        my_split = atomicAdd(&blk[0], 1u);
+        my_ovf = atomicAdd(&blk[1], sp.nseg - 1);
+      }
+    }
+  }
+  __syncthreads();
+  if constexpr (WH) {
+    if (tid < SEG_BINS && lh[tid]) atomicAdd(&work_hist[tid], lh[tid]);
+    if (tid == 0 && blk[0]) {
+      blk[2] = atomicAdd(&counters[0], blk[0]);
+      blk[3] = atomicAdd(&counters[1], blk[1]);
+    }
+    __syncthreads();
+    if (sp.nseg > 1) {
+      row_ovf_base[row] = blk[3] + my_ovf;
+      split_rows[blk[2] + my_split] = row;
+    }
+  }
   uint32_t* vi = val_idx + (size_t)ws * n;
   if (cached) {
 #pragma unroll
diff --git a/webgpu-msm-bls12-377_amd/csrc/sequencer.hip b/webgpu-msm-bls12-377_amd/csrc/sequencer.hip
--- a/webgpu-msm-bls12-377_amd/csrc/sequencer.hip
+++ b/webgpu-msm-bls12-377_amd/csrc/sequencer.hip
@@ -270,7 +270,15 @@
   uint32_t* meta_block = ctx->d_work_meta;
   uint32_t* key_max = meta_block + (2 * SEG_BINS + 4);
   if (ph.front) {
-    hipLaunchKernelGGL(k_clear_words, dim3(1), dim3(256), 0, st, meta_block, META_BLOCK_WORDS, (uint32_t*)d_err, ph.clear_err ? 1u : 0u);
+    uint32_t chunks = MAX_SORT_BLOCKS / wc;
+    const uint64_t want_chunks = (n + 4095) / 4096;
+    if (chunks > want_chunks) chunks = (uint32_t)(want_chunks ? want_chunks : 1);
+    const uint64_t per_chunk = (n + chunks - 1) / chunks;
+    const bool fused_count = ctx->front_fold && ph.even && !glv && !wide && !narrow && !ph.short_bytes;
+    const uint32_t clear_words = META_BLOCK_WORDS + (fused_count ? wc * NRANGE * chunks : 0u);
+    static_assert(MSM377_NUM_WINDOWS <= MAX_SORT_BLOCKS, "every window slot has a chunk");
+    hipLaunchKernelGGL(k_clear_words, dim3(std::min<uint32_t>((clear_words + 1023) / 1024, 64u)), dim3(256), 0, st, meta_block, clear_words, (uint32_t*)d_err,
+                       ph.clear_err ? 1u : 0u);
     uint32_t* top_key_max = (!glv && !ph.even && wb + wc == MSM377_NUM_WINDOWS) ? key_max + (wc - 1) : nullptr;
     const uint64_t max_items = (uint64_t)wc * NB + entries / SEG;
     const bool quad_acc = std::is_same<BP, CV>::value && std::is_same<CV, TeDev>::value && narrow && !ph.table && max_items <= ctx->narrow_quad_items;
@@ -304,6 +312,9 @@
         hipLaunchKernelGGL(k_decompose_geom, dim3((unsigned)((n + 255) / 256)), dim3(256), 0, st, d_scalars, digits, n, L, NARROW_EVEN_SIGNED, wc, bias, d_err);
       } else if (glv)
         hipLaunchKernelGGL(k_decompose_glv, dim3((unsigned)((n_scalars + 255) / 256)), dim3(256), 0, st, d_scalars, digits, n_scalars, wb, wc, d_err);
+      else if (fused_count)
+        hipLaunchKernelGGL(k_decompose_count, dim3((unsigned)((per_chunk + DC_SCALARS - 1) / DC_SCALARS), chunks), dim3(DC_THREADS), 0, st, d_scalars, digits, range_counts, n,
+                           wb, wc, chunks, per_chunk, d_err);
       else
         hipLaunchKernelGGL(k_decompose, dim3((unsigned)((n + 255) / 256)), dim3(256), 0, st, d_scalars, digits, n, wb, wc, d_err, top_key_max, ph.even ? 1u : 0u);
       if (!ph.short_bytes)
@@ -322,7 +333,7 @@
       hipLaunchKernelGGL(k_wide_part1, dim3(WS_CHUNKS, WIDE_WINDOWS), dim3(1024), 0, st, (const uint32_t*)ctx->wide.digits, (const uint32_t*)wc, sort_temp, n, (uint32_t)ph.table_stride);
       hipLaunchKernelGGL(k_wide_part2, dim3(WS_COARSE, WIDE_WINDOWS), dim3(1024), 0, st, (const SortElem*)sort_temp, (const uint32_t*)wc, ctx->wide.temp);
       hipLaunchKernelGGL(k_local_sort_lds<SortElem>, dim3(WIDE_NRANGE, 1), dim3(256), 0, st, (const SortElem*)ctx->wide.temp, region_base, row_ptr, val_idx, entries,
-                         (const uint32_t*)nullptr, WIDE_NRANGE, NB);
+                         (const uint32_t*)nullptr, WIDE_NRANGE, NB, SEG, (uint32_t*)nullptr, (uint32_t*)nullptr, (uint32_t*)nullptr, (uint32_t*)nullptr);
       HIP_TRY(ctx, hipGetLastError());
     } else if (narrow) {
       StageTimer t(ctx, MSM377_STAGE_SORT, st);
@@ -331,31 +342,35 @@
       HIP_TRY(ctx, hipGetLastError());
     } else {
       StageTimer t(ctx, MSM377_STAGE_SORT, st);
-      uint32_t chunks = MAX_SORT_BLOCKS / wc;
-      const uint64_t want = (n + 4095) / 4096;
-      if (chunks > want) chunks = (uint32_t)(want ? want : 1);
-      const uint64_t per_chunk = (n + chunks - 1) / chunks;
-      if (ph.short_bytes)
+      const bool fold = ctx->front_fold;
+      if (fused_count) {
+      } else if (ph.short_bytes)
         hipLaunchKernelGGL(k_range_count<true>, dim3(chunks, wc), dim3(1024), 0, st, digits, range_counts, n, chunks, per_chunk, key_max);
       else
         hipLaunchKernelGGL(k_range_count<false>, dim3(chunks, wc), dim3(1024), 0, st, digits, range_counts, n, chunks, per_chunk, key_max);
       HIP_TRY(ctx, hipGetLastError());
-      hipLaunchKernelGGL(k_range_scan, dim3(wc), dim3(NRANGE), 0, st, range_counts, region_base, chunks);
-      HIP_TRY(ctx, hipGetLastError());
+      if (!fold) {
+        hipLaunchKernelGGL(k_range_scan, dim3(wc), dim3(NRANGE), 0, st, range_counts, region_base, chunks);
+        HIP_TRY(ctx, hipGetLastError());
+      }
       const bool packed = ctx->sort_elem == 4 && sort_elem_bytes(n, false) == 4;
       ctx->last_sort_elem = packed ? 4u : 8u;
-      auto partition_and_sort = [&](auto* temp) {
+      auto partition_and_sort = [&](auto* temp, auto uns, auto folded) {
         using E = std::remove_pointer_t<decltype(temp)>;
-        if (ph.short_bytes)
-          hipLaunchKernelGGL((k_partition_staged<E, true>), dim3(chunks, wc), dim3(1024), 0, st, digits, range_counts, temp, n, chunks, per_chunk, key_max);
-        else
-          hipLaunchKernelGGL((k_partition_staged<E, false>), dim3(chunks, wc), dim3(1024), 0, st, digits, range_counts, temp, n, chunks, per_chunk, key_max);
+        constexpr bool UNS = decltype(uns)::value, F = decltype(folded)::value;
+        hipLaunchKernelGGL((k_partition_staged<E, UNS, F>), dim3(chunks, wc), dim3(1024), 0, st, digits, range_counts, temp, n, chunks, per_chunk, key_max, region_base);
         const hipError_t e = hipGetLastError();
         if (e != hipSuccess) return e;
-        hipLaunchKernelGGL(k_local_sort_lds<E>, dim3(NRANGE, wc), dim3(256), 0, st, (const E*)temp, region_base, row_ptr, val_idx, n, key_max, NRANGE, NB);
+        hipLaunchKernelGGL((k_local_sort_lds<E, F>), dim3(NRANGE, wc), dim3(256), 0, st, (const E*)temp, region_base, row_ptr, val_idx, n, key_max, NRANGE, NB, SEG,
+                           meta_block, row_ovf_base, meta_block + 2 * SEG_BINS + 1, split_rows);
         return hipGetLastError();
       };
-      HIP_TRY(ctx, packed ? partition_and_sort(reinterpret_cast<SortElem4*>(sort_temp)) : partition_and_sort(sort_temp));
+      auto with_elem = [&](auto uns, auto folded) {
+        return packed ? partition_and_sort(reinterpret_cast<SortElem4*>(sort_temp), uns, folded) : partition_and_sort(sort_temp, uns, folded);
+      };
+      using T = std::true_type;
+      using N = std::false_type;
+      HIP_TRY(ctx, ph.short_bytes ? (fold ? with_elem(T{}, T{}) : with_elem(T{}, N{})) : (fold ? with_elem(N{}, T{}) : with_elem(N{}, N{})));
     }
 
     {
@@ -366,8 +381,10 @@
       uint32_t* cursor = meta + SEG_BINS;
       uint32_t* total = meta + 2 * SEG_BINS;
       uint32_t* counters = meta + 2 * SEG_BINS + 1;
-      hipLaunchKernelGGL(k_work_hist, dim3((rows + 1023) / 1024), dim3(1024), 0, st, row_ptr, L, rows, SEG, work_hist, row_ovf_base, counters, split_rows);
-      HIP_TRY(ctx, hipGetLastError());
+      if (!(ctx->front_fold && !wide && !narrow)) {
+        hipLaunchKernelGGL(k_work_hist, dim3((rows + 1023) / 1024), dim3(1024), 0, st, row_ptr, L, rows, SEG, work_hist, row_ovf_base, counters, split_rows);
+        HIP_TRY(ctx, hipGetLastError());
+      }
       hipLaunchKernelGGL(k_work_scatter, dim3((rows + 1023) / 1024), dim3(1024), 0, st, row_ptr, L, rows, SEG, (const uint32_t*)work_hist, cursor, total, work);
       HIP_TRY(ctx, hipGetLastError());
       if (ctx->before_accumulate) {
```

Result: no change. 2.336, median of 6 (-0.7%).
